# facebookresearch/CODD

Hardware: AMD Instinct MI355X
Metric: frames/sec full CODD forward @960x540 (whole job) (higher is better)
Workload: dtype f32 (split-bf16 MFMA operands, f32 accumulate; HITNet + context network + Fusion exact f32); 1 GPU; full CODD (HITNetMF + Motion/RAFT3D iters=16 + Fusion) 960x540 padded to 960x576, max_disp=320, one video per GPU, steady-state frames (idx>=1), synthetic stereo sequence, random-init weights; conv_precision=split, hip_graph=True, frames_per_gpu=311, prewarm_frames=150, side_streams=True, library=codd_amd/csrc/libcodd_hip.so, full=False

## Files before the change

### codd_amd/_abi.py

```python
import ctypes as C
import os

from . import build as _build

c_float_p = C.POINTER(C.c_float)


class View(C.Structure):
    _fields_ = [("ptr", C.c_void_p), ("ctot", C.c_int), ("coff", C.c_int)]


class XsView(C.Structure):
    _fields_ = [("ptr", C.c_void_p), ("c8", C.c_int), ("hp", C.c_int), ("wp", C.c_int), ("bt", C.c_int),
                ("bl", C.c_int), ("o8", C.c_int), ("terms", C.c_int)]


class ConvParams(C.Structure):
    _fields_ = [
        ("in0", View), ("in1", View), ("C0", C.c_int), ("C1", C.c_int),
        ("B", C.c_int), ("Hin", C.c_int), ("Win", C.c_int),
        ("wpacked", C.c_void_p), ("bias", C.c_void_p),
        ("res1", View), ("res2", View), ("post", View),
        ("out", C.c_void_p), ("out_ctot", C.c_int), ("out_coff", C.c_int),
        ("Cout", C.c_int), ("Hout", C.c_int), ("Wout", C.c_int),
        ("kh", C.c_int), ("kw", C.c_int), ("sy", C.c_int), ("sx", C.c_int),
        ("pad_t", C.c_int), ("pad_l", C.c_int), ("dil_y", C.c_int), ("dil_x", C.c_int),
        ("act", C.c_int), ("store_mode", C.c_int), ("mb", C.c_int), ("npb", C.c_int), ("nw", C.c_int), ("ck", C.c_int), ("layout", C.c_int),
        ("terms", C.c_int), ("pgw", C.c_int), ("cgw", C.c_int),
        ("xs", C.c_void_p), ("xs_c8", C.c_int), ("xs_hp", C.c_int), ("xs_wp", C.c_int),
        ("xs_bt", C.c_int), ("xs_bl", C.c_int), ("xs_o8", C.c_int),
        ("xso", C.c_void_p), ("xso_c8", C.c_int), ("xso_hp", C.c_int), ("xso_wp", C.c_int), ("xso_bt", C.c_int),
        ("xso_bl", C.c_int), ("xso_o8", C.c_int), ("xso_terms", C.c_int), ("ksplit", C.c_int), ("dil2", C.c_int), ("gate", C.c_int),
    ]


ACT = dict(none=0, lrelu=1, relu=2, sigmoid=3, tanh=4, mish=5, relu_ch0=6)




class RollParams(C.Structure):
    _fields_ = [("in0", View), ("in1", View), ("C0", C.c_int), ("C1", C.c_int),
                ("B", C.c_int), ("H", C.c_int), ("W", C.c_int), ("C", C.c_int), ("mode", C.c_int),
                ("wA", C.c_void_p), ("bA", C.c_void_p), ("wB", C.c_void_p), ("bB", C.c_void_p),
                ("actA", C.c_int), ("actB", C.c_int), ("residual", C.c_int),
                ("out", C.c_void_p), ("out_ctot", C.c_int), ("out_coff", C.c_int), ("cout_store", C.c_int),
                ("rh", C.c_int)]


_i, _f, _p, _ll = C.c_int, C.c_float, C.c_void_p, C.c_longlong

SIGNATURES = {
    "codd_abi_version": (_i, []),
    "codd_conv2d": (_i, [C.POINTER(ConvParams), _p]),
    "codd_conv2d_check": (_i, [C.POINTER(ConvParams)]),
    "codd_conv2d_multi": (_i, [C.POINTER(ConvParams), _i, _p]),
    "codd_roll_packed_size": (_ll, [_i, _i, _i]),
    "codd_roll_pack_weights": (_i, [_p, _p, _i, _i, _i, _i, _p]),
    "codd_conv_roll": (_i, [C.POINTER(RollParams), _p]),
    "codd_conv2d_packed_size": (_ll, [_i] * 6),
    "codd_conv2d_pack_weights": (_i, [_p, _p, _i, _i, _i, _i, _i, _i, _p]),
    "codd_tile_costvol_argmin": (_i, [_p, _p, _i, _i, _i, _i, _i, _i, _p, _i, _i, _p, _i, _i, _i, _p]),
    "codd_tile_warp_cost": (_i, [_p, _p, _i, _i, _i, _i, View, View, _i, _p, _p, _p]),
    "codd_hyp_upsample": (_i, [View, _i, _i, _i, _f, _p, _i, _i, _p]),
    "codd_hyp_select": (_i, [_p, View, View, _i, _i, _i, _p, _i, _i, _p]),
    "codd_instnorm": (_i, [_p, _i, _i, _i, _p, _p, _i, _p, _p]),
    "codd_instnorm_xs": (_i, [_p, _i, _i, _i, _i, _p, _p, _i, _i, _p, XsView, _p]),
    "codd_conv2d_pack_weights_ex": (_i, [_p, _p, _i, _i, _i, _i, _i, _i, _ll, _ll, _f, _p]),
    "codd_allpairs_corr": (_i, [_p, _p, _i, _i, _i, _i, _p, _p, _p, _p, _p, _p]),
    "codd_allpairs_corr_scratch": (_ll, [_i, _i, _i, _i]),
    "codd_avgpool2": (_i, [_p, _i, _i, _i, _p, _p]),
    "codd_induced_flow": (_i, [_p, _p, _i, _i, _i, _f, _f, _f, _f, _p, _p]),
    "codd_context_split": (_i, [_p, _i, _i, _p, _p, _p]),
    "codd_se3_identity": (_i, [_p, _ll, _p]),
    "codd_corr_lookup": (_i, [_p, _p, _p, _p, _p, _i, _i, _i, _i, _p, _p]),
    "codd_raft_geometry": (_i, [_p, _p, _p, _i, _i, _i, _f, _f, _f, _f, _p, _p, _p]),
    "codd_se3_gn_step": (_i, [_p, _p, _i, _p, _p, _p, _p, _i, _i, _i, _f, _f, _f, _f, _i, _f, _f, _p, _p]),
    "codd_se3_gn_scratch": (_ll, [_i, _i, _i, _i]),
    "codd_set_option": (_i, [_i, _i]),
    "codd_get_option": (_i, [_i]),
    "codd_se3_gn_step_heads": (_i, [_p, XsView, _p, _p, _p, _p, _i, _i, _i, _f, _f, _f, _f, _i, _f, _f, _p, _p, _p]),
    "codd_cvx_upsample": (_i, [_p, _p, _i, _i, _i, _i, _i, _p, _p]),
    "codd_cvx_upsample_se3_weight": (_i, [_p, _p, _p, _i, _i, _i, _p, _p, _p]),
    "codd_disp_to_depth": (_i, [_p, _ll, _f, _p, _p]),
    "codd_subsample": (_i, [_p, _i, _i, _i, _i, _i, _i, _p, _p]),
    "codd_splat": (_i, [_p, _p, _i, _i, _i, _i, _i, _p, _i, _p, _i, _i, _i, _i, _i, _f, _f, _f, _f, _f, _f,
                        _p, _p, _p, _p]),
    "codd_splat_scratch": (_ll, [_i, _i, _i, _f]),
    "codd_resize_bilinear": (_i, [_p, _i, _i, _i, _i, _i, _i, _i, _p, _i, _i, _i, _i, _p]),
    "codd_resize_bilinear_add": (_i, [_p, _i, _i, _i, _i, _i, _i, _i, _p, _i, _i, _i, _i, _p, _p]),
    "codd_add_relu": (_i, [_p, _p, _ll, _i, _p, _p]),
    "codd_copy_many": (_i, [_p, _p, _p, _i, _p]),
    "codd_timestamp": (_i, [_p, _p]),
    "codd_gru_gate_zr": (_i, [_p, _p, _p, _p, _p, _p, _i, _i, _p, _p, _p]),
    "codd_gru_gate_q": (_i, [_p, _p, _p, _p, _p, _p, _p, _i, _i, _p, _p]),
    "codd_gru_gate_zr_xs": (_i, [_p, _p, _p, _p, _p, _p, _i, _i, _i, _p, XsView, _p]),
    "codd_gru_gate_q_xs": (_i, [_p, _p, _p, _p, _p, _p, _p, _i, _i, _i, _p, XsView, _p]),
    "codd_fusion_cues_lr": (_i, [_p] * 6 + [_i] * 7 + [_p, _p, _i, _i, _p]),
    "codd_fusion_cues_fr": (_i, [_p, _p, _p, _p, _i, _i, _i, _i, _p, _p]),
    "codd_fusion_forget": (_i, [_p, _p, _p, _p, _i, _i, _i, _i, _p, _p, _p]),
    "codd_disp_metrics": (_i, [_p, _p, _i, _i, _i, _i, _i, _f, _f, _f, _p, _p, _p]),
    "codd_raft_geometry_lookup": (_i, [_p, _p, _p, _p, _p, _p, _p, _i, _i, _i, _f, _f, _f, _f, _p, _p, _p, _p]),
    "codd_raft_geometry_lookup_xs": (_i, [_p, _p, _p, _p, _p, _p, _p, _i, _i, _i, _f, _f, _f, _f, _p, XsView, XsView, _p]),
    "codd_conv2d_packed_size_quad": (C.c_longlong, [_i, _i, _i, _i, _i, _i]),
    "codd_conv2d_pack_weights_quad": (_i, [_p, _p, _i, _i, _i, _i, _i, _i, _p]),
    "codd_split_bf16_bytes": (_ll, [_i] * 5),
    "codd_split_bf16": (_i, [View, _i, View, _i, _i, _i, _i, _i, _i, _i, _i, _i, _i, _p, _p]),
    "codd_conv2d_packed_bytes_bf16": (_ll, [_i] * 7),
    "codd_conv2d_pack_weights_bf16": (_i, [_p, _p, _i, _i, _i, _i, _i, _i, _i, _ll, _ll, _f, _p]),
    "codd_fusion_select": (_i, [_i, _p, _p, _p, _i, _i, _i, _i, _i, _f, _p, _p]),
    "codd_gt_motion": (_i, [_p, _p, _p, _i, _p, _p, _p, _i, _i, _i, _i, _i, _p, _p, _p, _p, _p, _p]),
    "codd_tepe_metrics": (_i, [_p, _p, _p, _p, _p, _p, _p, _i, _i, _i, _i, _i, _f, _f, _f, _p, _p, _p]),
    "codd_sceneflow_metrics": (_i, [_p] * 6 + [_i] * 5 + [_f] * 7 + [_p, _p, _p]),
    "codd_preprocess": (_i, [_p, _i, _i, _i, C.POINTER(C.c_float), C.POINTER(C.c_float), _i, _i, _p, _p]),
    "codd_fusion_blend": (_i, [_p, _p, _p, _p, _i, _i, _i, _i, _p, _p, _p, _p]),
}

ABI_VERSION = 12
_lib = None
LOADED = None
MISSING = []


class CoddHipError(RuntimeError):
    pass


def lib_path():
    ab = os.environ.get("CODD_LIB_AB")
    if ab:
        import sys
        print(f"codd_amd: WARNING: CODD_LIB_AB is set -- loading the prebuilt {ab} instead of the in-tree library; it is NOT "
              f"checked against the sources of this tree", file=sys.stderr, flush=True)
        return ab
    return _build.LIB


def load():
    global _lib, LOADED
    if _lib is not None:
        return _lib
    path = lib_path()
    if path == _build.LIB and (not os.path.exists(path) or _build.needs_build()):
        import fcntl
        try:
            lock = open(os.path.join(os.path.dirname(path), ".build.lock"), "w")
        except OSError as e:
            raise CoddHipError(f"libcodd_hip.so is missing or older than its sources and {os.path.dirname(path)} is "
                               f"not writable: {e}") from e
        with lock:
            fcntl.flock(lock, fcntl.LOCK_EX)
            try:
                if not os.path.exists(path) or _build.needs_build():
                    try:
                        _build.build(verbose=False)
                    except Exception as e:
                        raise CoddHipError(f"libcodd_hip.so is missing or older than its sources and the rebuild "
                                           f"failed: {e}") from e
            finally:
                fcntl.flock(lock, fcntl.LOCK_UN)
    lib = C.CDLL(path)
    for name, (res, args) in SIGNATURES.items():
        try:
            fn = getattr(lib, name)
        except AttributeError:
            MISSING.append(name)
            continue
        fn.restype = res
        fn.argtypes = args
    if lib.codd_abi_version() != ABI_VERSION:
        raise CoddHipError("ABI version mismatch")
    _lib, LOADED = lib, path
    return lib


OPTIONS = dict(gn_q4=0, gn_builder=1)


def set_option(name, value):
    rc = load().codd_set_option(OPTIONS[name], int(value))
    if rc < 0:
        raise CoddHipError(f"codd_set_option({name}, {value}) rejected")
    return rc


def check(rc, what):
    if rc != 0:
        raise CoddHipError(f"{what} failed with code {rc}")
```

### codd_amd/csrc/conv.hip

```cpp
#include "conv_quad_kernel.h"
#include <stdio.h>
#include <stdlib.h>

CONV_ALL_GROUPS(CONV_DECLARE)
CONVQ_ALL(CONVQ_DECLARE)
CONVQ_MULTI(CONVQM_DECLARE)


__global__ void conv_pack_kernel(const float* __restrict__ w, float* __restrict__ wp, int Cout, int Cin, int ntaps,
                                 int mb, int ck, int wrow, int nchunks, long long total, long long co_stride,
                                 long long ci_stride, float scale) {
  long long e = (long long)blockIdx.x * blockDim.x + threadIdx.x;
  if (e >= total) return;
  int col = (int)(e % wrow);
  long long t = e / wrow;
  int c = (int)(t % ck); t /= ck;
  int tap = (int)(t % ntaps); t /= ntaps;
  int chunk = (int)(t % nchunks);
  int cog = (int)(t / nchunks);
  int co = cog * 16 * mb + col, ci = chunk * ck + c;
  float v = 0.f;
  if (col < 16 * mb && co < Cout && ci < Cin) v = w[(size_t)co * co_stride + (size_t)ci * ci_stride + tap] * scale;
  wp[e] = v;
}

__global__ void conv_pack_quad_kernel(const float* __restrict__ w, float* __restrict__ wp, int Cout, int Cin, int ntaps,
                                      int mb, int ck, int nchunks, long long total) {
  long long e = (long long)blockIdx.x * blockDim.x + threadIdx.x;
  if (e >= total) return;
  const int q = (int)(e & 3);
  long long t = e >> 2;
  const int col = (int)(t % (16 * mb)); t /= 16 * mb;
  const int cq = (int)(t % (ck >> 2)); t /= ck >> 2;
  const int tap = (int)(t % ntaps); t /= ntaps;
  const int chunk = (int)(t % nchunks);
  const int cog = (int)(t / nchunks);
  const int co = cog * 16 * mb + col, ci = chunk * ck + 4 * cq + q;
  wp[e] = (co < Cout && ci < Cin) ? w[((size_t)co * Cin + ci) * ntaps + tap] : 0.f;
}

extern "C" long long codd_conv2d_packed_size_quad(int Cout, int Cin, int kh, int kw, int mb, int ck) {
  if (mb < 1 || !(ck == 16 || ck == 32)) return -1;
  return (long long)cdiv(Cout, 16 * mb) * cdiv(Cin, ck) * (kh * kw) * ck * 16 * mb;
}

extern "C" int codd_conv2d_pack_weights_quad(const float* w, float* wpacked, int Cout, int Cin, int kh, int kw, int mb,
                                             int ck, void* stream) {
  const long long total = codd_conv2d_packed_size_quad(Cout, Cin, kh, kw, mb, ck);
  if (total <= 0 || !w || !wpacked) return CODD_EINVAL;
  conv_pack_quad_kernel<<<cdiv(total, 256), 256, 0, (hipStream_t)stream>>>(w, wpacked, Cout, Cin, kh * kw, mb, ck,
                                                                           cdiv(Cin, ck), total);
  CODD_LAUNCH_CHECK();
  return CODD_OK;
}

static inline int wrow_of(int mb) { return 16 * mb + ((mb & 1) ? 0 : 16); }

extern "C" long long codd_conv2d_packed_size(int Cout, int Cin, int kh, int kw, int mb, int ck) {
  if (mb < 1 || ck < 4 || (ck & 3)) return -1;
  long long ncog = cdiv(Cout, 16 * mb), nchunks = cdiv(Cin, ck);
  return ncog * nchunks * (long long)(kh * kw) * ck * wrow_of(mb);
}

extern "C" int codd_conv2d_pack_weights_ex(const float* w, float* wpacked, int Cout, int Cin, int kh, int kw, int mb,
                                           int ck, long long co_stride, long long ci_stride, float scale,
                                           void* stream) {
  long long total = codd_conv2d_packed_size(Cout, Cin, kh, kw, mb, ck);
  if (total <= 0 || !w || !wpacked) return CODD_EINVAL;
  int nchunks = cdiv(Cin, ck);
  conv_pack_kernel<<<cdiv(total, 256), 256, 0, (hipStream_t)stream>>>(w, wpacked, Cout, Cin, kh * kw, mb, ck,
                                                                      wrow_of(mb), nchunks, total, co_stride,
                                                                      ci_stride, scale);
  CODD_LAUNCH_CHECK();
  return CODD_OK;
}

extern "C" int codd_conv2d_pack_weights(const float* w, float* wpacked, int Cout, int Cin, int kh, int kw, int mb,
                                        int ck, void* stream) {
  return codd_conv2d_pack_weights_ex(w, wpacked, Cout, Cin, kh, kw, mb, ck, (long long)Cin * kh * kw,
                                     (long long)kh * kw, 1.f, stream);
}

template <int NW, int NPB, int MB, int WREG, int IREG>
static int launch_conv(const ConvK& k, size_t lds, int grid, hipStream_t s) {
  if (lds > 64 * 1024) {
    hipError_t e = hipFuncSetAttribute((const void*)conv_mfma_kernel<NW, NPB, MB, WREG, IREG>,
                                       hipFuncAttributeMaxDynamicSharedMemorySize, (int)lds);
    if (e != hipSuccess) return (int)e;
  }
  conv_mfma_kernel<NW, NPB, MB, WREG, IREG><<<grid, NW * 64, lds, s>>>(k);
  CODD_LAUNCH_CHECK();
  return CODD_OK;
}

template <int NPB, int MB>
static int launch_conv_regs(const ConvK& k, size_t lds, int grid, hipStream_t s) {
  const int wr = cdiv(k.wchunk >> 2, 256), ir = cdiv(k.nunits, 256);
  if (wr <= 4 && ir <= 4) return launch_conv<4, NPB, MB, 4, 4>(k, lds, grid, s);
  if (wr <= 4 && ir <= 8) return launch_conv<4, NPB, MB, 4, 8>(k, lds, grid, s);
  if (wr <= 12 && ir <= 4) return launch_conv<4, NPB, MB, 12, 4>(k, lds, grid, s);
  if (wr <= 12 && ir <= 8) return launch_conv<4, NPB, MB, 12, 8>(k, lds, grid, s);
  if (wr <= 16 && ir <= 8) return launch_conv<4, NPB, MB, 16, 8>(k, lds, grid, s);
  return CODD_EUNSUPPORTED;
}

template <int NW, int MB>
static int launch_conv_nwx(const ConvK& k, size_t lds, int grid, hipStream_t s) {
  const int wr = cdiv(k.wchunk >> 2, NW * 64), ir = cdiv(k.nunits, NW * 64);
  if (wr <= 8 && ir <= 4) return launch_conv<NW, 1, MB, 8, 4>(k, lds, grid, s);
  if (wr <= 16 && ir <= 4) return launch_conv<NW, 1, MB, 16, 4>(k, lds, grid, s);
  return CODD_EUNSUPPORTED;
}

template <int NW, int NPB, int MB, int WREG, int QREG>
static int launch_quad(const ConvK& k, size_t lds, int grid, hipStream_t s) {
  if (lds > 64 * 1024) {
    hipError_t e = hipFuncSetAttribute((const void*)conv_quad_kernel<NW, NPB, MB, WREG, QREG>,
                                       hipFuncAttributeMaxDynamicSharedMemorySize, (int)lds);
    if (e != hipSuccess) return (int)e;
  }
  conv_quad_kernel<NW, NPB, MB, WREG, QREG><<<grid, NW * 64, lds, s>>>(k);
  CODD_LAUNCH_CHECK();
  return CODD_OK;
}

static int launch_quad_any(const ConvK& k, int nw, size_t lds, int grid, hipStream_t s) {
  const codd_conv_params& p = k.p;
  const int nt = nw * 64, wr = cdiv(k.wchunk >> 2, nt), qr = cdiv((p.ck >> 2) * k.upc, nt);
#define Q(W, N, M, R, QQ) if (nw == W && p.npb == N && p.mb == M && wr <= R && qr <= QQ) return launch_quad<W, N, M, R, QQ>(k, lds, grid, s);
  Q(4, 1, 1, 8, 2) Q(4, 1, 2, 8, 1) Q(4, 1, 2, 16, 2) Q(4, 1, 4, 12, 1) Q(4, 1, 4, 16, 2)
  Q(4, 2, 1, 8, 2) Q(4, 2, 2, 8, 2) Q(4, 2, 2, 16, 2) Q(4, 2, 4, 12, 2) Q(4, 2, 4, 16, 2)
  Q(4, 4, 1, 8, 4) Q(4, 4, 2, 8, 4)
  Q(9, 1, 1, 8, 1) Q(9, 1, 2, 8, 1) Q(9, 1, 4, 8, 1) Q(9, 1, 4, 16, 1)
#undef Q
  return CODD_EUNSUPPORTED;
}

int codd_conv2d_bf16(const codd_conv_params* pp, void* stream, int dry_run);

extern "C" int codd_conv2d_check(const codd_conv_params* pp) {
  if (!pp || pp->layout != 2) return CODD_EINVAL;
  return codd_conv2d_bf16(pp, nullptr, 1);
}

static int conv_fill(const codd_conv_params* pp, ConvK& k, size_t& lds, long long& grid, int& nw) {
  k.p = *pp;
  const codd_conv_params& p = k.p;
  if (!p.in0.ptr || !p.out || !p.wpacked || p.C0 <= 0 || p.C1 < 0 || (p.C1 > 0 && !p.in1.ptr)) return CODD_EINVAL;
  if (p.ck < 4 || (p.ck & 3) || p.B < 1 || p.Cout < 1 || p.kh < 1 || p.kw < 1 || p.pad_l < 0 || p.pad_t < 0)
    return CODD_EINVAL;
  if (!(p.mb == 1 || p.mb == 2 || p.mb == 4) || !(p.npb == 1 || p.npb == 2 || p.npb == 4)) return CODD_EINVAL;
  if (p.store_mode && (p.kh != 1 || p.kw != 1 || p.res1.ptr || p.res2.ptr || p.post.ptr)) return CODD_EUNSUPPORTED;
  k.cin = p.C0 + p.C1;
  k.nchunks = cdiv(k.cin, p.ck);
  k.ntaps = p.kh * p.kw;
  const int xb = p.npb >= 2 ? 2 : 1, rpw = p.npb / xb;
  nw = p.nw ? p.nw : 4;
  if (nw != 4 && (!(nw == 9 || nw == 2 || nw == 8) || p.npb != 1)) return CODD_EUNSUPPORTED;
  k.th = nw * rpw;
  k.tw = 16 * xb;
  k.thi = (k.th - 1) * p.sy + (p.kh - 1) * p.dil_y + 1;
  k.twi = (k.tw - 1) * p.sx + (p.kw - 1) * p.dil_x + 1;
  k.xoff = (4 - (p.pad_l % 4)) % 4;
  k.twp = ((k.xoff + k.twi + 3) / 4) * 4;
  k.twp4 = k.twp / 4;
  k.upc = k.thi * k.twp4;
  k.nunits = p.ck * k.upc;
  const int per = k.thi * k.twp;
  if (p.sx == 1) k.chs = ((per + 15) / 32) * 32 + 16;
  else k.chs = per + 4;
  k.wrow = wrow_of(p.mb);
  k.wchunk = k.ntaps * p.ck * k.wrow;
  k.tiles_x = cdiv(p.Wout, k.tw);
  k.tiles_y = cdiv(p.Hout, k.th);
  k.cout_eff = p.store_mode ? 4 * p.Cout : p.Cout;
  k.ncog = cdiv(k.cout_eff, 16 * p.mb);
  const size_t hwb = (size_t)p.Hin * p.Win * sizeof(float);
  k.vec_ok = (p.Win % 4 == 0) && ((uintptr_t)p.in0.ptr % 16 == 0) && (hwb % 16 == 0) &&
             (p.C1 == 0 || (uintptr_t)p.in1.ptr % 16 == 0);
  lds = ((size_t)k.wchunk + (size_t)p.ck * k.chs) * sizeof(float);
  if (p.layout == 1) {
    if (!(p.ck == 16 || p.ck == 32) || p.sx > 2 || !k.vec_ok) return CODD_EUNSUPPORTED;
    k.wchunk = k.ntaps * p.ck * 16 * p.mb;
    lds = ((size_t)k.wchunk + (size_t)p.ck * k.thi * k.twp) * sizeof(float);
  } else if (p.layout != 0) {
    return CODD_EINVAL;
  }
  if (lds > 160 * 1024) return CODD_EUNSUPPORTED;
  grid = (long long)k.tiles_x * k.tiles_y * k.ncog * p.B;
  if (grid <= 0 || grid > 0x7fffffffLL) return CODD_EINVAL;
  k.xcd = 1;
  return CODD_OK;
}

extern "C" int codd_conv2d(const codd_conv_params* pp, void* stream) {
  if (!pp) return CODD_EINVAL;
  if (pp->layout != 2 && (pp->dil2 || pp->gate)) return CODD_EUNSUPPORTED;
  if (pp->layout == 2) {
    const codd_conv_params& q = *pp;
    if (!q.xs || (!q.out && !q.xso) || !q.wpacked || q.C0 <= 0 || q.C1 < 0 || q.B < 1 || q.Cout < 1 || q.kh < 1 || q.kw < 1 ||
        q.pad_l < 0 || q.pad_t < 0)
      return CODD_EINVAL;
    if (q.store_mode && (q.kh != 1 || q.kw != 1 || q.res1.ptr || q.res2.ptr || q.post.ptr)) return CODD_EUNSUPPORTED;
    return codd_conv2d_bf16(pp, stream, 0);
  }
  ConvK k;
  size_t lds;
  long long grid;
  int nw;
  const int rc = conv_fill(pp, k, lds, grid, nw);
  if (rc != CODD_OK) return rc;
  const codd_conv_params& p = k.p;
  hipStream_t s = (hipStream_t)stream;
  if (p.layout == 1) return launch_quad_any(k, nw, lds, (int)grid, s);
#define CASEW(W, M) if (nw == W && p.mb == M) return launch_conv_nwx<W, M>(k, lds, (int)grid, s)
  CASEW(9, 1); CASEW(9, 2); CASEW(9, 4); CASEW(2, 1); CASEW(2, 2); CASEW(2, 4); CASEW(8, 1); CASEW(8, 2); CASEW(8, 4);
#undef CASEW
#define CASE(N, M) if (p.npb == N && p.mb == M) return launch_conv_regs<N, M>(k, lds, (int)grid, s)
  CASE(1, 1); CASE(1, 2); CASE(1, 4);
  CASE(2, 1); CASE(2, 2); CASE(2, 4);
  CASE(4, 1); CASE(4, 2); CASE(4, 4);
#undef CASE
  return CODD_EUNSUPPORTED;
}

template <int NW, int NPB, int MB, int WREG, int QREG>
static int launch_quad_multi(const ConvKN& kn, size_t lds, int grid, hipStream_t s) {
  if (lds > 64 * 1024) {
    hipError_t e = hipFuncSetAttribute((const void*)conv_quad_multi_kernel<NW, NPB, MB, WREG, QREG>,
                                       hipFuncAttributeMaxDynamicSharedMemorySize, (int)lds);
    if (e != hipSuccess) return (int)e;
  }
  conv_quad_multi_kernel<NW, NPB, MB, WREG, QREG><<<grid, NW * 64, lds, s>>>(kn);
  CODD_LAUNCH_CHECK();
  return CODD_OK;
}

extern "C" int codd_conv2d_multi(const codd_conv_params* ps, int n, void* stream) {
  if (!ps || n < 1 || n > CONVQ_MULTI_MAX) return CODD_EINVAL;
  if (n == 1) return codd_conv2d(ps, stream);
  ConvKN kn;
  memset(&kn, 0, sizeof(kn));
  size_t lds = 0;
  long long total = 0;
  int wr = 0, qr = 0;
  for (int i = 0; i < n; ++i) {
    size_t l;
    long long g;
    int nw;
    if (ps[i].layout != 1) return CODD_EUNSUPPORTED;
    const int rc = conv_fill(&ps[i], kn.k[i], l, g, nw);
    if (rc != CODD_OK) return rc;
    const codd_conv_params& p = kn.k[i].p;
    if (nw != 4 || p.npb != 1 || p.mb != ps[0].mb || !(p.mb == 1 || p.mb == 2)) return CODD_EUNSUPPORTED;
    const int w_ = cdiv(kn.k[i].wchunk >> 2, 256), q_ = cdiv((p.ck >> 2) * kn.k[i].upc, 256);
    wr = w_ > wr ? w_ : wr;
    qr = q_ > qr ? q_ : qr;
    lds = l > lds ? l : lds;
    kn.start[i] = (int)total;
    total += g;
  }
  for (int i = n; i <= CONVQ_MULTI_MAX; ++i) kn.start[i] = (int)total;
  if (total > 0x7fffffffLL) return CODD_EINVAL;
  hipStream_t s = (hipStream_t)stream;
  if (ps[0].mb == 1 && wr <= 8 && qr <= 2) return launch_quad_multi<4, 1, 1, 8, 2>(kn, lds, (int)total, s);
  if (ps[0].mb == 2 && wr <= 16 && qr <= 2) return launch_quad_multi<4, 1, 2, 16, 2>(kn, lds, (int)total, s);
  return CODD_EUNSUPPORTED;
}

extern "C" int codd_avgpool2(const float* in, int BC, int h, int w, float* out, void* stream);

#define CORR_MB 4
#define CORR_CK 32
extern "C" long long codd_allpairs_corr_scratch(int B, int D, int h, int w) {
  long long packed = codd_conv2d_packed_size(h * w, D, 1, 1, CORR_MB, CORR_CK);
  long long pooled = 0;
  int hh = h, ww = w;
  for (int i = 1; i < 4; ++i) { hh >>= 1; ww >>= 1; pooled += (long long)D * hh * ww; }
  return (long long)B * (packed + pooled);
}

extern "C" int codd_allpairs_corr(const float* f1, const float* f2, int B, int D, int h, int w, float* lvl0,
                                  float* lvl1, float* lvl2, float* lvl3, float* scratch, void* stream) {
  if (!f1 || !f2 || !lvl0 || !lvl1 || !lvl2 || !lvl3 || !scratch || (h >> 3) < 1 || (w >> 3) < 1) return CODD_EINVAL;
  const int N = h * w;
  const long long packed = codd_conv2d_packed_size(N, D, 1, 1, CORR_MB, CORR_CK);
  float* lv[4] = {lvl0, lvl1, lvl2, lvl3};
  for (int b = 0; b < B; ++b) {
    float* wp = scratch + (size_t)b * packed;
    int rc = codd_conv2d_pack_weights_ex(f1 + (size_t)b * D * N, wp, N, D, 1, 1, CORR_MB, CORR_CK, 1, N, 1.f / 16.f,
                                         stream);
    if (rc) return rc;
  }
  float* pool = scratch + (size_t)B * packed;
  const float* src = f2;
  int hh = h, ww = w;
  for (int i = 0; i < 4; ++i) {
    if (i > 0) {
      int rc = codd_avgpool2(src, B * D, hh, ww, pool, stream);
      if (rc) return rc;
      src = pool;
      hh >>= 1; ww >>= 1;
      pool += (size_t)B * D * hh * ww;
    }
    for (int b = 0; b < B; ++b) {
      codd_conv_params p;
      memset(&p, 0, sizeof(p));
      p.in0.ptr = src + (size_t)b * D * hh * ww; p.in0.ctot = D; p.in0.coff = 0;
      p.C0 = D; p.C1 = 0; p.B = 1; p.Hin = hh; p.Win = ww;
      p.wpacked = scratch + (size_t)b * packed;
      p.out = lv[i] + (size_t)b * N * hh * ww; p.out_ctot = N; p.out_coff = 0;
      p.Cout = N; p.Hout = hh; p.Wout = ww;
      p.kh = p.kw = 1; p.sy = p.sx = 1; p.dil_y = p.dil_x = 1;
      p.act = CODD_ACT_NONE; p.mb = CORR_MB; p.ck = CORR_CK;
      p.npb = 1;
      int rc = codd_conv2d(&p, stream);
      if (rc) return rc;
    }
  }
  return CODD_OK;
}
```

### codd_amd/csrc/conv_bf16_kernel.h

```cpp
#pragma once
#include <stdlib.h>
#include "conv_kernel.h"

typedef __bf16 bf16x8 __attribute__((ext_vector_type(8)));
typedef _Float16 f16x8 __attribute__((ext_vector_type(8)));

struct ConvB {
  codd_conv_params p;
  int cin, nchunks, ntaps, noct;
  int nk;
  int th, tw, thi, twi;
  int pu, xb;
  int npix;
  int xplane;
  int nring;
  int os16;
  int iplane16;
  int ibuf16;
  int wplane16;
  int nco;
  int wslots;
  int tiles_x, tiles_y, ncog, cout_eff;
  int khe;
  unsigned m_iplane16, m_os16, m_twi, m_noct, m_kw;
};
static inline unsigned convb_magic(int d) { return d <= 1 ? 0u : (unsigned)((0x100000000ULL + (unsigned)d - 1) / (unsigned)d); }
__device__ __forceinline__ int convb_div(int n, unsigned M, int d) { return d == 1 ? n : (int)__umulhi((unsigned)n, M); }

constexpr int CONVB_NWP = 4;
constexpr int CONVB_MAXP = 6;
#ifdef CONVB_NO_DMA
#define CONVB_DMA_N(n) 0
#else
#define CONVB_DMA_N(n) (n)
#endif
#ifdef CONVB_NO_INPUT
#define CONVB_IN_N(n) 0
#else
#define CONVB_IN_N(n) (n)
#endif

static inline int convb_geometry(const codd_conv_params* pp, ConvB& k, size_t& lds, long long& grid, bool need_xs) {
  k.p = *pp;
  const codd_conv_params& p = k.p;
  if (p.ck < 8 || (p.ck & 7) || !CODD_TERMS_OK(p.terms) || p.nw < 1 || p.npb < 1 || p.npb > 2 ||
      p.pgw < 1 || p.cgw < 1 || p.mb < 1 || p.mb % p.cgw)
    return CODD_EINVAL;
  const int planes = CODD_TERMS_PLANES(p.terms);
  k.cin = p.C0 + p.C1;
  k.ntaps = p.kh * p.kw;
  k.noct = p.ck >> 3;
  k.nchunks = cdiv(k.cin, p.ck);
  k.nk = cdiv((long long)k.ntaps * k.noct, 4);
  k.th = p.nw; k.xb = p.npb; k.pu = k.th * k.xb; k.tw = 16 * k.xb;
  if (p.dil2 < 0 || (p.dil2 > 0 && ((p.kh & 1) || !(p.kh / 2 & 1) || !(p.kw & 1) || p.dil2 > p.dil_y || p.dil2 > p.dil_x)))
    return CODD_EINVAL;
  k.khe = p.dil2 > 0 ? p.kh / 2 : p.kh;
  k.thi = (k.th - 1) * p.sy + (k.khe - 1) * p.dil_y + 1;
  k.twi = (k.tw - 1) * p.sx + (p.kw - 1) * p.dil_x + 1;
  k.npix = k.thi * k.twi;
  k.os16 = ((k.npix + 15) / 16) * 16;
  while ((planes * k.noct * k.os16) & 63) k.os16 += 16;
  k.iplane16 = k.noct * k.os16;
  k.ibuf16 = planes * k.iplane16;
  k.nco = 16 * p.mb;
  k.wplane16 = k.nk * 4 * k.nco;
  k.wslots = planes * k.wplane16;
  k.tiles_x = cdiv(p.Wout, k.tw);
  k.tiles_y = cdiv(p.Hout, k.th);
  k.cout_eff = p.store_mode ? 4 * p.Cout : p.Cout;
  k.ncog = cdiv(k.cout_eff, k.nco);
  const size_t per = ((size_t)k.wslots + (size_t)k.ibuf16) * 16, tab = ((size_t)k.nk + 2) * 16;
  k.nring = (k.nchunks >= 3 && 3 * per + tab <= 160 * 1024) ? 3 : 2;
  lds = k.nring * per + tab;
  if (lds > 160 * 1024) return CODD_EUNSUPPORTED;
  if (p.ksplit < 0 || p.ksplit > 2) return CODD_EINVAL;
  if (p.ksplit == 2 && (size_t)cdiv(k.pu, p.pgw) * p.mb * p.pgw * 1024 > k.nring * per) return CODD_EUNSUPPORTED;
  if ((k.nring - 1) * (cdiv(k.wslots >> 6, CONVB_NWP) + cdiv(k.ibuf16 >> 6, CONVB_NWP)) > 56) return CODD_EUNSUPPORTED;
  k.xplane = p.xs_c8 * p.xs_hp * p.xs_wp;
  if (k.nring * (k.wslots + k.ibuf16) + 64 >= 65536 || (k.nk + 2) * 4 >= 65536) return CODD_EUNSUPPORTED;
  k.m_iplane16 = convb_magic(k.iplane16); k.m_os16 = convb_magic(k.os16); k.m_twi = convb_magic(k.twi);
  k.m_noct = convb_magic(k.noct); k.m_kw = convb_magic(p.kw);
  if (need_xs && (!p.xs || p.xs_o8 < 0 || p.xs_c8 < p.xs_o8 + k.nchunks * k.noct || p.xs_bt < p.pad_t ||
                  p.xs_bl < p.pad_l || p.xs_hp < p.xs_bt + p.Hin || p.xs_wp < p.xs_bl + p.Win ||
                  p.xs_hp < p.xs_bt - p.pad_t + (k.tiles_y * k.th - 1) * p.sy + (k.khe - 1) * p.dil_y + 1 ||
                  p.xs_wp < p.xs_bl - p.pad_l + (k.tiles_x * k.tw - 1) * p.sx + (p.kw - 1) * p.dil_x + 1))
    return CODD_EINVAL;
  if (p.gate < 0 || p.gate > 3) return CODD_EINVAL;
  if (need_xs && p.gate) {
    const int G = p.gate == 2 ? k.cout_eff / 3 : k.cout_eff;
    auto c4ok = [](const codd_view& v, int need) {
      return v.ptr && !((uintptr_t)v.ptr & 15) && !(v.ctot & 3) && !(v.coff & 3) && v.coff >= 0 && v.coff + need <= v.ctot;
    };
    if (p.store_mode || (G & 15) || (p.gate == 2 && 3 * G != k.cout_eff)) return CODD_EUNSUPPORTED;
    if (!p.out || ((uintptr_t)p.out & 15) || (p.out_ctot & 3) || (p.out_coff & 3) ||
        p.out_coff + (p.gate == 2 ? 2 * G : G) > p.out_ctot || (p.bias && ((uintptr_t)p.bias & 15)))
      return CODD_EINVAL;
    if (p.gate == 1 && (p.xso || p.res1.ptr || p.res2.ptr || p.post.ptr)) return CODD_EUNSUPPORTED;
    if (p.gate == 2 && (!p.xso || !c4ok(p.res1, 3 * G) || !c4ok(p.res2, 2 * G) || !c4ok(p.post, G))) return CODD_EINVAL;
    if (p.gate == 3 && (!p.xso || !c4ok(p.res1, 2 * G) || !c4ok(p.post, G) || p.res2.ptr)) return CODD_EINVAL;
    if (p.xso && (p.xso_terms != p.terms || p.xso_o8 < 0 || p.xso_bt < 0 || p.xso_bl < 0 ||
                  p.xso_c8 < p.xso_o8 + cdiv(G, 8) || p.xso_hp < p.xso_bt + p.Hout || p.xso_wp < p.xso_bl + p.Wout))
      return CODD_EINVAL;
  } else if (need_xs && p.xso) {
    if (p.store_mode || p.res1.ptr || p.res2.ptr || p.post.ptr || p.act == CODD_ACT_RELU_CH0) return CODD_EUNSUPPORTED;
    if (p.bias && ((uintptr_t)p.bias & 15)) return CODD_EINVAL;
    if (p.xso_terms != p.terms || p.xso_o8 < 0 || p.xso_bt < 0 || p.xso_bl < 0 ||
        p.xso_c8 < p.xso_o8 + cdiv(k.cout_eff, 8) || p.xso_hp < p.xso_bt + p.Hout || p.xso_wp < p.xso_bl + p.Wout)
      return CODD_EINVAL;
  }
  grid = (long long)k.tiles_x * k.tiles_y * k.ncog * p.B;
  if (grid <= 0 || grid > 0x7fffffffLL) return CODD_EINVAL;
  return CODD_OK;
}

__device__ __attribute__((noinline)) f32x4 convb_act_slow(f32x4 v, int act) {
#pragma unroll
  for (int r = 0; r < 4; ++r) v[r] = act_apply(v[r], act, 1);
  return v;
}
__device__ __forceinline__ f32x4 convb_act(f32x4 v, int act, int co) {
  if (act == CODD_ACT_NONE) return v;
  if (act == CODD_ACT_RELU || (act == CODD_ACT_RELU_CH0 && co == 0)) {
#pragma unroll
    for (int r = 0; r < 4; ++r) v[r] = fmaxf(v[r], 0.f);
    return v;
  }
  if (act == CODD_ACT_RELU_CH0) return v;
  if (act == CODD_ACT_LRELU02) {
#pragma unroll
    for (int r = 0; r < 4; ++r) v[r] = v[r] > 0.f ? v[r] : 0.2f * v[r];
    return v;
  }
  return convb_act_slow(v, act);
}

__device__ __forceinline__ void convb_wait_vmcnt(int n) {
#define CONVB_W1(N) case N: asm volatile("s_waitcnt vmcnt(" #N ")" ::: "memory"); break;
#define CONVB_W8(N) CONVB_W1(N) CONVB_W1(N + 1) CONVB_W1(N + 2) CONVB_W1(N + 3) CONVB_W1(N + 4) CONVB_W1(N + 5) CONVB_W1(N + 6) CONVB_W1(N + 7)
  switch (n) {
    CONVB_W8(0) CONVB_W8(8) CONVB_W8(16) CONVB_W8(24) CONVB_W8(32) CONVB_W8(40) CONVB_W8(48)
    default: break;
  }
#undef CONVB_W8
#undef CONVB_W1
}

__device__ __forceinline__ void convb_dma16(const uint4* gsrc, unsigned lds_dst) {
  unsigned keep;
  asm volatile("s_mov_b32 %0, m0\n\ts_mov_b32 m0, %2\n\ts_nop 0\n\tglobal_load_lds_dwordx4 %1, off\n\ts_mov_b32 m0, %0"
               : "=&s"(keep) : "v"(gsrc), "s"(lds_dst) : "memory");
}

template <int I, int NR, int NM>
struct ConvbSched {
  static __device__ __forceinline__ void run() {
    constexpr int q = ((I + 1) * NM) / NR - (I * NM) / NR;
    if constexpr (q > 0) __builtin_amdgcn_sched_group_barrier(0x008, q, 0);
    __builtin_amdgcn_sched_group_barrier(0x100, 1, 0);
    if constexpr (I + 1 < NR) ConvbSched<I + 1, NR, NM>::run();
  }
};

template <int PGW, int CGW, int A, int B, int TERMS, int OUTF, int KS>
__global__ __launch_bounds__((PGW * CGW * KS + CONVB_NWP) * 64) void conv_bf16_kernel(const ConvB k) {
  constexpr int NWT = PGW * CGW;
  constexpr int NWC = NWT * KS;
  constexpr int NTP = CONVB_NWP * 64;
  constexpr int NPL = CODD_TERMS_PLANES(TERMS);
  constexpr bool F16 = CODD_TERMS_IS_F16(TERMS);
  extern __shared__ __attribute__((aligned(16))) uint4 smem4[];
  uint4* wl = smem4;
  uint4* il = smem4 + k.nring * k.wslots;
  int* etab = (int*)(il + k.nring * k.ibuf16);
  const codd_conv_params& p = k.p;
  const int tid = threadIdx.x, lane = tid & 63;
  const int wave = __builtin_amdgcn_readfirstlane(tid >> 6);

  int bid = blockIdx.x;
  const int tx = bid % k.tiles_x; bid /= k.tiles_x;
  const int ty = bid % k.tiles_y; bid /= k.tiles_y;
  const int cog = bid % k.ncog;
  const int b = bid / k.ncog;

  if (wave >= NWC) {
    const int pt = tid - NWC * 64;
    const int pw = wave - NWC;
    const int nwv = k.wslots >> 6, niv = k.ibuf16 >> 6;
    const int nd = (nwv - pw + CONVB_NWP - 1) / CONVB_NWP + (niv - pw + CONVB_NWP - 1) / CONVB_NWP;
    const unsigned wl_lds = (unsigned)(uintptr_t)(__attribute__((address_space(3))) uint4*)wl;
    const unsigned il_lds = (unsigned)(uintptr_t)(__attribute__((address_space(3))) uint4*)il;
#define BF_DMA_W(CH, BUF)                                                                                 \
  {                                                                                                       \
    const uint4* wsrc_ = (const uint4*)p.wpacked + ((size_t)(cog * k.nchunks + (CH))) * k.wslots + lane;  \
    const unsigned wdst_ = wl_lds + (unsigned)(BUF) * (unsigned)k.wslots * 16u;                           \
    for (int i_ = pw; i_ < nwv; i_ += CONVB_NWP)                                                          \
      convb_dma16(wsrc_ + i_ * 64, __builtin_amdgcn_readfirstlane(wdst_ + (unsigned)i_ * 1024u));         \
  }
#ifndef CONVB_NO_PRODUCER
    BF_DMA_W(0, 0);
#endif
    const int oct_rec = p.xs_hp * p.xs_wp;
    const uint4* xs0 = (const uint4*)p.xs + (size_t)b * NPL * k.xplane + (size_t)p.xs_o8 * oct_rec +
                       (size_t)(ty * k.th * p.sy + p.xs_bt - p.pad_t) * p.xs_wp + tx * k.tw * p.sx + p.xs_bl - p.pad_l;
    auto piece_off = [&](int i_) -> int {
      const int s_ = i_ * 64 + lane;
      const int pl_ = convb_div(s_, k.m_iplane16, k.iplane16), r_ = s_ - pl_ * k.iplane16;
      const int oc_ = convb_div(r_, k.m_os16, k.os16);
      int px_ = r_ - oc_ * k.os16;
      px_ = px_ < k.npix ? px_ : 0;
      const int y_ = convb_div(px_, k.m_twi, k.twi), x_ = px_ - y_ * k.twi;
      return pl_ * k.xplane + oc_ * oct_rec + y_ * p.xs_wp + x_;
    };
    int ioff[CONVB_MAXP];
#pragma unroll
    for (int q_ = 0; q_ < CONVB_MAXP; ++q_) ioff[q_] = piece_off(pw + q_ * CONVB_NWP);
#define BF_DMA_I(CH, BUF)                                                                                 \
  {                                                                                                       \
    const uint4* xsrc_ = xs0 + (size_t)(CH) * k.noct * oct_rec;                                           \
    const unsigned idst_ = il_lds + (unsigned)(BUF) * (unsigned)k.ibuf16 * 16u;                           \
    _Pragma("unroll") for (int q_ = 0; q_ < CONVB_MAXP; ++q_) {                                           \
      const int i_ = pw + q_ * CONVB_NWP;                                                                 \
      if (i_ < niv) convb_dma16(xsrc_ + ioff[q_], __builtin_amdgcn_readfirstlane(idst_ + (unsigned)i_ * 1024u)); \
    }                                                                                                     \
    for (int i_ = pw + CONVB_MAXP * CONVB_NWP; i_ < niv; i_ += CONVB_NWP)                                 \
      convb_dma16(xsrc_ + piece_off(i_), __builtin_amdgcn_readfirstlane(idst_ + (unsigned)i_ * 1024u));   \
  }
#define BF_DMA(CH, BUF) { BF_DMA_W(CH, BUF) BF_DMA_I(CH, BUF) }
#ifndef CONVB_NO_PRODUCER
    const int ahead = k.nring - 1;
    BF_DMA_I(0, 0);
    if (ahead > 1 && k.nchunks > 1) BF_DMA(1, 1);
#endif
    for (int e = pt; e < (k.nk + 2) * 4; e += NTP) {
      const int tap = convb_div(e, k.m_noct, k.noct), oct = e - tap * k.noct;
      int off = 0;
      if (e < k.nk * 4 && tap < k.ntaps) {
        const int ky = convb_div(tap, k.m_kw, p.kw), kx = tap - ky * p.kw;
        if (p.dil2 > 0 && ky < k.khe)
          off = oct * k.os16 + ((k.khe >> 1) * (p.dil_y - p.dil2) + ky * p.dil2) * k.twi +
                (p.kw >> 1) * (p.dil_x - p.dil2) + kx * p.dil2;
        else
          off = oct * k.os16 + (ky - (p.dil2 > 0 ? k.khe : 0)) * p.dil_y * k.twi + kx * p.dil_x;
      }
      etab[e] = off;
    }
#ifndef CONVB_NO_PRODUCER
    convb_wait_vmcnt(ahead > 1 && k.nchunks > 1 ? nd : 0);
    asm volatile("s_waitcnt lgkmcnt(0)" ::: "memory");
    __builtin_amdgcn_s_barrier();
    int slot = ahead == k.nring ? 0 : ahead;
    for (int c = 0; c < k.nchunks; ++c) {
      if (c + ahead < k.nchunks) BF_DMA(c + ahead, slot);
      slot = slot + 1 == k.nring ? 0 : slot + 1;
      int fly_ = k.nchunks - (c + 2);
      fly_ = fly_ < 0 ? 0 : (fly_ > ahead - 1 ? ahead - 1 : fly_);
      convb_wait_vmcnt(fly_ * nd);
      __builtin_amdgcn_s_barrier();
    }
#endif
#undef BF_DMA
#undef BF_DMA_W
#undef BF_DMA_I
    return;
  }

  const int g = lane >> 4, j = lane & 15;
  const int kpart = KS == 1 ? 0 : wave / NWT, wset = KS == 1 ? wave : wave - kpart * NWT;
  const int cgi = wset % CGW, pgi = wset / CGW;
  f32x4 acc[A][B];
#pragma unroll
  for (int a = 0; a < A; ++a)
#pragma unroll
    for (int m = 0; m < B; ++m) acc[a][m] = (f32x4){0.f, 0.f, 0.f, 0.f};

  int pbase[A];
#pragma unroll
  for (int a = 0; a < A; ++a) {
    int u = pgi * A + a;
    if (u >= k.pu) u = k.pu - 1;
    const int prow = u / k.xb, pcol = (u - prow * k.xb) * 16 + j;
    pbase[a] = prow * p.sy * k.twi + pcol * p.sx;
  }
  const int woff = g * k.nco + cgi * B * 16 + j;
  const int wstep = 4 * k.nco;

  struct Frag { bf16x8 ah[B], al[B], bh[A], bl[A]; };
#define BF_LOAD(F, KSTP)                                                                                   \
  {                                                                                                       \
    const int eo_ = eo;                                                                                   \
    eo = etab[((KSTP) + KS) * 4 + g];                                                                   \
    const uint4* wp_ = wb + woff + (KSTP) * wstep;                                                          \
    _Pragma("unroll") for (int m_ = 0; m_ < B; ++m_) {                                                    \
      F.ah[m_] = __builtin_bit_cast(bf16x8, wp_[m_ * 16]);                                                \
      if (NPL == 2) F.al[m_] = __builtin_bit_cast(bf16x8, wp_[k.wplane16 + m_ * 16]);                   \
    }                                                                                                     \
    _Pragma("unroll") for (int a_ = 0; a_ < A; ++a_) {                                                    \
      F.bh[a_] = __builtin_bit_cast(bf16x8, ib[eo_ + pbase[a_]]);                                         \
      if (NPL == 2) F.bl[a_] = __builtin_bit_cast(bf16x8, ib[k.iplane16 + eo_ + pbase[a_]]);            \
    }                                                                                                     \
  }
  auto mma = [](bf16x8 x, bf16x8 y, f32x4 c) -> f32x4 {
    if constexpr (F16)
      return __builtin_amdgcn_mfma_f32_16x16x32_f16(__builtin_bit_cast(f16x8, x), __builtin_bit_cast(f16x8, y), c, 0, 0, 0);
    else
      return __builtin_amdgcn_mfma_f32_16x16x32_bf16(x, y, c, 0, 0, 0);
  };
#define BF_MFMA(F)                                                                                        \
  {                                                                                                       \
    if (NPL == 2) {                                                                                       \
      _Pragma("unroll") for (int a = 0; a < A; ++a) _Pragma("unroll") for (int m = 0; m < B; ++m)         \
        acc[a][m] = OUTF ? mma(F.al[m], F.bh[a], acc[a][m]) : mma(F.bh[a], F.al[m], acc[a][m]);           \
      _Pragma("unroll") for (int a = 0; a < A; ++a) _Pragma("unroll") for (int m = 0; m < B; ++m)         \
        acc[a][m] = OUTF ? mma(F.ah[m], F.bl[a], acc[a][m]) : mma(F.bl[a], F.ah[m], acc[a][m]);           \
    }                                                                                                     \
    _Pragma("unroll") for (int a = 0; a < A; ++a) _Pragma("unroll") for (int m = 0; m < B; ++m)           \
      acc[a][m] = OUTF ? mma(F.ah[m], F.bh[a], acc[a][m]) : mma(F.bh[a], F.ah[m], acc[a][m]);             \
  }

  __syncthreads();
#ifndef CONVB_NO_CONSUMER
  const int klast = k.nk - 1;
  constexpr int NRD = 1 + NPL * (A + B), NMF = (NPL == 2 ? 3 : 1) * A * B;
  int wsel = 0;
  for (int ch = 0; ch < k.nchunks; ++ch) {
    const uint4* wb = wl + wsel * k.wslots;
    const uint4* ib = il + wsel * k.ibuf16;
    wsel = wsel + 1 == k.nring ? 0 : wsel + 1;
    const int kfirst = KS == 1 ? 0 : ((kpart + ch) & 1);
    if (KS == 1 || kfirst < k.nk) {
      const int mylast = KS == 1 ? klast : kfirst + ((klast - kfirst) / KS) * KS;
      Frag f0, f1;
      int eo = etab[kfirst * 4 + g];
      BF_LOAD(f0, kfirst);
      int ks = kfirst;
      for (; ks + KS < k.nk; ks += 2 * KS) {
#ifdef CONVB_NO_LDSREAD
        if (ch == 0 && ks == kfirst)
#endif
        BF_LOAD(f1, ks + KS);
        BF_MFMA(f0);
#ifndef CONVB_NO_SCHED
        ConvbSched<0, NRD, NMF>::run();
#endif
#ifdef CONVB_NO_LDSREAD
        if (ch == 0 && ks == kfirst)
#endif
        BF_LOAD(f0, ks + 2 * KS < mylast ? ks + 2 * KS : mylast);
        BF_MFMA(f1);
#ifndef CONVB_NO_SCHED
        ConvbSched<0, NRD, NMF>::run();
#endif
      }
      if (ks < k.nk) BF_MFMA(f0);
    }
#ifndef CONVB_NO_BARRIER
    __syncthreads();
#endif
  }
#endif
#undef BF_LOAD
#undef BF_MFMA
  if constexpr (KS == 2) {
    f32x4* red = (f32x4*)smem4 + (size_t)wset * (A * B) * 64 + lane;
#pragma unroll
    for (int a = 0; a < A; ++a)
#pragma unroll
      for (int m = 0; m < B; ++m)
        if (((a * B + m) & 1) != kpart) red[(a * B + m) * 64] = acc[a][m];
    __syncthreads();
#pragma unroll
    for (int a = 0; a < A; ++a)
#pragma unroll
      for (int m = 0; m < B; ++m)
        if (((a * B + m) & 1) == kpart) acc[a][m] += red[(a * B + m) * 64];
  }

#ifdef CONVB_NO_EPILOGUE
  {
    float s_ = 0.f;
#pragma unroll
    for (int a = 0; a < A; ++a)
#pragma unroll
      for (int m = 0; m < B; ++m) s_ += acc[a][m][0] + acc[a][m][1] + acc[a][m][2] + acc[a][m][3];
    p.out[(size_t)blockIdx.x * 256 + tid] = s_;
    return;
  }
#endif
  if constexpr (OUTF == 1) {
    const int orec = p.xso_hp * p.xso_wp;
    uint4* xo = (uint4*)p.xso + (size_t)b * NPL * p.xso_c8 * orec;
    const bool odd = g & 1;
#pragma unroll
    for (int a = 0; a < A; ++a) {
      const int u = pgi * A + a;
      const int prow = u / k.xb;
      const int oy = ty * k.th + prow;
      const int ox = tx * k.tw + (u - prow * k.xb) * 16 + j;
      const bool inb = u < k.pu && oy < p.Hout && ox < p.Wout;
#pragma unroll
      for (int m = 0; m < B; ++m) {
        if (KS == 2 && ((a * B + m) & 1) != kpart) continue;
        const int co0 = (cog * CGW * B + cgi * B + m) * 16 + 4 * g;
        f32x4 v = acc[a][m];
        if (p.bias) {
          if (co0 + 3 < k.cout_eff) v += *(const f32x4*)(p.bias + co0);
          else
#pragma unroll
            for (int r = 0; r < 4; ++r) v[r] += co0 + r < k.cout_eff ? p.bias[co0 + r] : 0.f;
        }
        int rco = co0;
        if (p.gate) {
          const int hw_ = p.Hout * p.Wout, pix_ = oy * p.Wout + ox;
          auto c4 = [&](const float* base, int ctot, int c) {
            return (f32x4*)(base + (((size_t)b * (ctot >> 2) + (c >> 2)) * hw_ + pix_) * 4);
          };
          const bool live = inb && co0 < k.cout_eff;
          const int ctile = co0 & ~15;
          if (p.gate == 1) {
            if (live) *c4(p.out, p.out_ctot, p.out_coff + co0) = v;
            continue;
          }
          const int G = p.gate == 2 ? k.cout_eff / 3 : k.cout_eff;
          if (p.gate == 2) {
            if (live) v += *c4(p.res1.ptr, p.res1.ctot, p.res1.coff + co0);
            if (ctile >= 2 * G) {
              if (live) *c4(p.out, p.out_ctot, p.out_coff + co0 - G) = v;
              continue;
            }
            if (live) v += *c4(p.res2.ptr, p.res2.ctot, p.res2.coff + co0);
            v = convb_act_slow(v, CODD_ACT_SIGMOID);
            if (ctile < G) {
              if (live) *c4(p.out, p.out_ctot, p.out_coff + co0) = v;
              continue;
            }
            rco = co0 - G;
            if (live) v *= *c4(p.post.ptr, p.post.ctot, p.post.coff + rco);
          } else {
            f32x4 z = f32x4{0.f, 0.f, 0.f, 0.f}, h = z;
            if (live) {
              v += *c4(p.res1.ptr, p.res1.ctot, p.res1.coff + G + co0);
              z = *c4(p.res1.ptr, p.res1.ctot, p.res1.coff + co0);
              h = *c4(p.post.ptr, p.post.ctot, p.post.coff + co0);
            }
            v = convb_act_slow(v, CODD_ACT_TANH);
#pragma unroll
            for (int r = 0; r < 4; ++r) v[r] = (1.f - z[r]) * h[r] + z[r] * v[r];
            if (live) *c4(p.out, p.out_ctot, p.out_coff + co0) = v;
          }
        } else {
          v = convb_act(v, p.act, 1);
        }
#pragma unroll
        for (int r = 0; r < 4; ++r) v[r] = co0 + r < k.cout_eff ? v[r] : 0.f;
        unsigned hi2[2], lo2[2];
#pragma unroll
        for (int q = 0; q < 2; ++q) {
          if constexpr (F16) {
            const _Float16 h0 = (_Float16)v[2 * q], h1 = (_Float16)v[2 * q + 1];
            const _Float16 l0 = (_Float16)(v[2 * q] - (float)h0), l1 = (_Float16)(v[2 * q + 1] - (float)h1);
            hi2[q] = (unsigned)__builtin_bit_cast(unsigned short, h0) | ((unsigned)__builtin_bit_cast(unsigned short, h1) << 16);
            lo2[q] = (unsigned)__builtin_bit_cast(unsigned short, l0) | ((unsigned)__builtin_bit_cast(unsigned short, l1) << 16);
          } else {
            const __bf16 h0 = (__bf16)v[2 * q], h1 = (__bf16)v[2 * q + 1];
            const __bf16 l0 = (__bf16)(v[2 * q] - (float)h0), l1 = (__bf16)(v[2 * q + 1] - (float)h1);
            hi2[q] = (unsigned)__builtin_bit_cast(unsigned short, h0) | ((unsigned)__builtin_bit_cast(unsigned short, h1) << 16);
            lo2[q] = (unsigned)__builtin_bit_cast(unsigned short, l0) | ((unsigned)__builtin_bit_cast(unsigned short, l1) << 16);
          }
        }
        const unsigned s0 = odd ? hi2[0] : lo2[0], s1 = odd ? hi2[1] : lo2[1];
        const unsigned r0 = __shfl_xor(s0, 16, 64), r1 = __shfl_xor(s1, 16, 64);
        const uint4 rec = odd ? make_uint4(r0, r1, lo2[0], lo2[1]) : make_uint4(hi2[0], hi2[1], r0, r1);
        const int oct = (rco >> 3) + p.xso_o8;
        if (inb && (co0 & ~7) < k.cout_eff && (!odd || NPL == 2))
          xo[(size_t)(odd ? p.xso_c8 * orec : 0) + ((size_t)oct * p.xso_hp + oy + p.xso_bt) * p.xso_wp + ox + p.xso_bl] = rec;
      }
    }
    return;
  }
  const int hwout = p.Hout * p.Wout;
  const bool vec = (p.Wout & 3) == 0 && p.store_mode == 0;
#pragma unroll
  for (int a = 0; a < A; ++a) {
    const int u = pgi * A + a;
    if (u >= k.pu) continue;
    const int prow = u / k.xb;
    const int oy = ty * k.th + prow;
    const int ox = tx * k.tw + (u - prow * k.xb) * 16 + 4 * g;
    if (oy >= p.Hout || ox >= p.Wout) continue;
    const int pix = oy * p.Wout + ox;
#pragma unroll
    for (int m = 0; m < B; ++m) {
      if (KS == 2 && ((a * B + m) & 1) != kpart) continue;
      const int co = (cog * CGW * B + cgi * B + m) * 16 + j;
      if (co >= k.cout_eff) continue;
      f32x4 v = acc[a][m];
      if (p.store_mode == 0) {
        if (p.bias) v += p.bias[co];
        float* op = p.out + ((size_t)b * p.out_ctot + p.out_coff + co) * (size_t)hwout + pix;
        if (vec) {
          if (p.res1.ptr) v += *(const f32x4*)(view_ptr(p.res1, b, co, hwout) + pix);
          if (p.res2.ptr) v += *(const f32x4*)(view_ptr(p.res2, b, co, hwout) + pix);
          v = convb_act(v, p.act, co);
          if (p.post.ptr) v += *(const f32x4*)(view_ptr(p.post, b, co, hwout) + pix);
#if defined(CONVB_NT_STORE)
          __builtin_nontemporal_store(v, (f32x4*)op);
#elif defined(CONVB_SC1_STORE)
          asm volatile("global_store_dwordx4 %0, %1, off sc1" ::"v"(op), "v"(v) : "memory");
#else
          *(f32x4*)op = v;
#endif
        } else {
#pragma unroll
          for (int r = 0; r < 4; ++r)
            if (ox + r < p.Wout) {
              if (p.res1.ptr) v[r] += view_ptr(p.res1, b, co, hwout)[pix + r];
              if (p.res2.ptr) v[r] += view_ptr(p.res2, b, co, hwout)[pix + r];
            }
          v = convb_act(v, p.act, co);
#pragma unroll
          for (int r = 0; r < 4; ++r)
            if (ox + r < p.Wout) op[r] = v[r] + (p.post.ptr ? view_ptr(p.post, b, co, hwout)[pix + r] : 0.f);
        }
      } else {
        const int q = co / p.Cout, c = co - q * p.Cout;
        if (p.bias) v += p.bias[c];
        v = convb_act(v, p.act, c);
        const int W2 = 2 * p.Wout;
        float* op = p.out + ((size_t)b * p.out_ctot + p.out_coff + c) * (size_t)(4 * hwout) +
                    (size_t)(2 * oy + (q >> 1)) * W2 + (q & 1);
#pragma unroll
        for (int r = 0; r < 4; ++r)
          if (ox + r < p.Wout) op[2 * (ox + r)] = v[r];
      }
    }
  }
}

#define CONVB_GROUP_A(X) X(2, 2, 5, 2, 1)
#define CONVB_GROUP_B(X) X(4, 1, 4, 4, 1)
#define CONVB_GROUP_C(X) X(4, 1, 4, 2, 1)
#define CONVB_GROUP_D(X) X(4, 1, 4, 1, 1) X(4, 1, 8, 1, 1)
#define CONVB_GROUP_E(X) X(4, 1, 2, 2, 1) X(4, 1, 2, 1, 1)
#define CONVB_GROUP_F(X) X(4, 1, 3, 4, 1) X(4, 1, 3, 2, 1)
#define CONVB_GROUP_G(X) X(2, 2, 5, 2, 2)
#define CONVB_GROUP_H(X) X(4, 1, 4, 2, 2)
#define CONVB_GROUP_I(X) X(4, 1, 3, 2, 2) X(4, 1, 3, 4, 2)
#define CONVB_GROUP_J(X) X(4, 2, 4, 2, 1)
#define CONVB_GROUP_K(X) X(4, 2, 3, 2, 1)
#define CONVB_GROUP_L(X) X(8, 1, 4, 4, 1)
#define CONVB_ALL(X)                                                                                   \
  CONVB_GROUP_A(X) CONVB_GROUP_B(X) CONVB_GROUP_C(X) CONVB_GROUP_D(X) CONVB_GROUP_E(X) CONVB_GROUP_F(X) \
  CONVB_GROUP_G(X) CONVB_GROUP_H(X) CONVB_GROUP_I(X) CONVB_GROUP_J(X) CONVB_GROUP_K(X) CONVB_GROUP_L(X)
#define CONVB_DECLARE(PGW, CGW, A, B, KS)                                                        \
  extern template __global__ void conv_bf16_kernel<PGW, CGW, A, B, 1, 0, KS>(const ConvB);      \
  extern template __global__ void conv_bf16_kernel<PGW, CGW, A, B, 3, 0, KS>(const ConvB);      \
  extern template __global__ void conv_bf16_kernel<PGW, CGW, A, B, 1, 1, KS>(const ConvB);      \
  extern template __global__ void conv_bf16_kernel<PGW, CGW, A, B, 3, 1, KS>(const ConvB);      \
  extern template __global__ void conv_bf16_kernel<PGW, CGW, A, B, 16, 0, KS>(const ConvB);     \
  extern template __global__ void conv_bf16_kernel<PGW, CGW, A, B, 16, 1, KS>(const ConvB);     \
  extern template __global__ void conv_bf16_kernel<PGW, CGW, A, B, 48, 0, KS>(const ConvB);     \
  extern template __global__ void conv_bf16_kernel<PGW, CGW, A, B, 48, 1, KS>(const ConvB);
#define CONVB_DEFINE(PGW, CGW, A, B, KS)                                                         \
  template __global__ void conv_bf16_kernel<PGW, CGW, A, B, 1, 0, KS>(const ConvB);             \
  template __global__ void conv_bf16_kernel<PGW, CGW, A, B, 3, 0, KS>(const ConvB);             \
  template __global__ void conv_bf16_kernel<PGW, CGW, A, B, 1, 1, KS>(const ConvB);             \
  template __global__ void conv_bf16_kernel<PGW, CGW, A, B, 3, 1, KS>(const ConvB);             \
  template __global__ void conv_bf16_kernel<PGW, CGW, A, B, 16, 0, KS>(const ConvB);            \
  template __global__ void conv_bf16_kernel<PGW, CGW, A, B, 16, 1, KS>(const ConvB);            \
  template __global__ void conv_bf16_kernel<PGW, CGW, A, B, 48, 0, KS>(const ConvB);            \
  template __global__ void conv_bf16_kernel<PGW, CGW, A, B, 48, 1, KS>(const ConvB);
```

### codd_amd/csrc/conv_kernel.h

```cpp
#pragma once
#include "common.h"
#include <stdint.h>
#include <string.h>


struct ConvK {
  codd_conv_params p;
  int cin, nchunks, ntaps;
  int th, tw, thi, twi, chs;
  int wrow, wchunk;
  int tiles_x, tiles_y, ncog;
  int cout_eff;
  int twp;
  int xoff;
  int twp4;
  int upc;
  int nunits;
  int vec_ok;
  int xcd;
};

__device__ __forceinline__ int conv_xcd_item(int bid, int nwg) {
  const int q = nwg >> 3, r = nwg & 7, x = bid & 7, idx = bid >> 3;
  return (x < r ? x * (q + 1) : r * (q + 1) + (x - r) * q) + idx;
}

__device__ __forceinline__ const float* view_ptr(const codd_view& v, int b, int c, int hw) {
  return v.ptr + ((size_t)b * v.ctot + v.coff + c) * (size_t)hw;
}

template <int NW, int NPB, int MB, int WREG, int IREG>
__global__ __launch_bounds__(NW * 64) void conv_mfma_kernel(const ConvK k) {
  constexpr int NT = NW * 64;
  extern __shared__ __attribute__((aligned(16))) float smem[];
  float* wl = smem;
  float* il = smem + k.wchunk;
  const codd_conv_params& p = k.p;
  const int tid = threadIdx.x, lane = tid & 63, wave = tid >> 6;
  const int g = lane >> 4, j = lane & 15;
  constexpr int XB = NPB >= 2 ? 2 : 1;
  constexpr int RPW = NPB / XB;

  int bid = k.xcd ? conv_xcd_item(blockIdx.x, gridDim.x) : blockIdx.x;
  const int tx = bid % k.tiles_x; bid /= k.tiles_x;
  const int ty = bid % k.tiles_y; bid /= k.tiles_y;
  const int cog = bid % k.ncog;
  const int b = bid / k.ncog;

  const int hwin = p.Hin * p.Win;
  const int gy0 = ty * k.th * p.sy - p.pad_t;
  const int gxs = tx * k.tw * p.sx - p.pad_l - k.xoff;

  int u_lds[IREG], u_g[IREG], u_c[IREG];
  unsigned u_m[IREG];
#pragma unroll
  for (int r = 0; r < IREG; ++r) {
    const int u = tid + r * NT;
    u_c[r] = -1; u_m[r] = 0; u_lds[r] = 0; u_g[r] = 0;
    if (u < k.nunits) {
      const int c = u / k.upc, rem = u - c * k.upc;
      const int y = rem / k.twp4, x4 = rem - y * k.twp4;
      const int gy = gy0 + y, gx = gxs + 4 * x4;
      unsigned m = 0;
      if ((unsigned)gy < (unsigned)p.Hin) {
#pragma unroll
        for (int q = 0; q < 4; ++q) m |= ((unsigned)(gx + q) < (unsigned)p.Win) ? (1u << q) : 0u;
      }
      u_c[r] = c; u_m[r] = m;
      u_lds[r] = c * k.chs + y * k.twp + 4 * x4;
      u_g[r] = gy * p.Win + gx;
    }
  }
  const int wchunk4 = k.wchunk >> 2;
  float4 wreg[WREG], ireg[IREG];

#define CONV_ISSUE(CH)                                                                                    \
  {                                                                                                       \
    const float4* src_ = (const float4*)(p.wpacked + ((size_t)(cog * k.nchunks + (CH))) * k.wchunk);      \
    _Pragma("unroll") for (int r = 0; r < WREG; ++r) {                                                    \
      const int e = tid + r * NT;                                                                         \
      wreg[r] = e < wchunk4 ? src_[e] : make_float4(0.f, 0.f, 0.f, 0.f);                                  \
    }                                                                                                     \
    const int c0_ = (CH) * p.ck;                                                                          \
    _Pragma("unroll") for (int r = 0; r < IREG; ++r) {                                                    \
      float4 v = make_float4(0.f, 0.f, 0.f, 0.f);                                                         \
      const int cg = c0_ + u_c[r];                                                                        \
      if (u_c[r] >= 0 && cg < k.cin && u_m[r]) {                                                          \
        const float* s_ =                                                                                 \
            (cg < p.C0 ? view_ptr(p.in0, b, cg, hwin) : view_ptr(p.in1, b, cg - p.C0, hwin)) + u_g[r];    \
        if (u_m[r] == 0xFu && k.vec_ok) {                                                                 \
          v = *(const float4*)s_;                                                                         \
        } else {                                                                                          \
          if (u_m[r] & 1u) v.x = s_[0];                                                                   \
          if (u_m[r] & 2u) v.y = s_[1];                                                                   \
          if (u_m[r] & 4u) v.z = s_[2];                                                                   \
          if (u_m[r] & 8u) v.w = s_[3];                                                                   \
        }                                                                                                 \
      }                                                                                                   \
      ireg[r] = v;                                                                                        \
    }                                                                                                     \
  }
#define CONV_COMMIT()                                                                                     \
  {                                                                                                       \
    float4* dst_ = (float4*)wl;                                                                           \
    _Pragma("unroll") for (int r = 0; r < WREG; ++r) {                                                    \
      const int e = tid + r * NT;                                                                         \
      if (e < wchunk4) dst_[e] = wreg[r];                                                                 \
    }                                                                                                     \
    _Pragma("unroll") for (int r = 0; r < IREG; ++r) if (u_c[r] >= 0) *(float4*)(il + u_lds[r]) = ireg[r]; \
  }

  f32x4 acc[NPB][MB];
#pragma unroll
  for (int a = 0; a < NPB; ++a)
#pragma unroll
    for (int m = 0; m < MB; ++m) acc[a][m] = (f32x4){0.f, 0.f, 0.f, 0.f};

  int pbase[NPB];
#pragma unroll
  for (int a = 0; a < NPB; ++a) {
    const int prow = wave * RPW + a / XB, pcol = (a % XB) * 16 + j;
    pbase[a] = prow * p.sy * k.twp + pcol * p.sx + k.xoff;
  }

  CONV_ISSUE(0);
  for (int ch = 0; ch < k.nchunks; ++ch) {
    __syncthreads();
    CONV_COMMIT();
    __syncthreads();
    if (ch + 1 < k.nchunks) CONV_ISSUE(ch + 1);
    for (int ky = 0; ky < p.kh; ++ky) {
      for (int kx = 0; kx < p.kw; ++kx) {
        const float* wp = wl + (ky * p.kw + kx) * p.ck * k.wrow + j + g * k.wrow;
        const float* ip = il + ky * p.dil_y * k.twp + kx * p.dil_x + g * k.chs;
        const int wstep = 4 * k.wrow, istep = 4 * k.chs;
#pragma unroll 4
        for (int c4 = 0; c4 < p.ck; c4 += 4) {
          float av[MB], bv[NPB];
#pragma unroll
          for (int m = 0; m < MB; ++m) av[m] = wp[m * 16];
#pragma unroll
          for (int a = 0; a < NPB; ++a) bv[a] = ip[pbase[a]];
          wp += wstep;
          ip += istep;
#pragma unroll
          for (int a = 0; a < NPB; ++a)
#pragma unroll
            for (int m = 0; m < MB; ++m)
              acc[a][m] = __builtin_amdgcn_mfma_f32_16x16x4f32(av[m], bv[a], acc[a][m], 0, 0, 0);
        }
      }
    }
  }

  const int hwout = p.Hout * p.Wout;
#pragma unroll
  for (int a = 0; a < NPB; ++a) {
    const int oy = ty * k.th + wave * RPW + a / XB;
    const int ox = tx * k.tw + (a % XB) * 16 + j;
    if (oy >= p.Hout || ox >= p.Wout) continue;
    const int pix = oy * p.Wout + ox;
#pragma unroll
    for (int m = 0; m < MB; ++m) {
#pragma unroll
      for (int r = 0; r < 4; ++r) {
        const int co = (cog * MB + m) * 16 + 4 * g + r;
        if (co >= k.cout_eff) continue;
        float v = acc[a][m][r];
        if (p.store_mode == 0) {
          if (p.bias) v += p.bias[co];
          if (p.res1.ptr) v += view_ptr(p.res1, b, co, hwout)[pix];
          if (p.res2.ptr) v += view_ptr(p.res2, b, co, hwout)[pix];
          v = act_apply(v, p.act, co);
          if (p.post.ptr) v += view_ptr(p.post, b, co, hwout)[pix];
          p.out[((size_t)b * p.out_ctot + p.out_coff + co) * (size_t)hwout + pix] = v;
        } else {
          const int q = co / p.Cout, c = co - q * p.Cout;
          if (p.bias) v += p.bias[c];
          v = act_apply(v, p.act, c);
          const int W2 = 2 * p.Wout;
          p.out[((size_t)b * p.out_ctot + p.out_coff + c) * (size_t)(4 * hwout) +
                (size_t)(2 * oy + (q >> 1)) * W2 + 2 * ox + (q & 1)] = v;
        }
      }
    }
  }
}

#define CONV_REGS_NW4(X, NPB, MB) X(4, NPB, MB, 4, 4) X(4, NPB, MB, 4, 8) X(4, NPB, MB, 12, 4) X(4, NPB, MB, 12, 8) X(4, NPB, MB, 16, 8)
#define CONV_REGS_NWX(X, NW, MB) X(NW, 1, MB, 8, 4) X(NW, 1, MB, 16, 4)
#define CONV_GROUP_0(X) CONV_REGS_NW4(X, 1, 1)
#define CONV_GROUP_1(X) CONV_REGS_NW4(X, 1, 2)
#define CONV_GROUP_2(X) CONV_REGS_NW4(X, 1, 4)
#define CONV_GROUP_3(X) CONV_REGS_NW4(X, 2, 1) CONV_REGS_NW4(X, 2, 2)
#define CONV_GROUP_4(X) CONV_REGS_NW4(X, 2, 4) CONV_REGS_NW4(X, 4, 1)
#define CONV_GROUP_5(X) CONV_REGS_NW4(X, 4, 2)
#define CONV_GROUP_6(X) CONV_REGS_NW4(X, 4, 4)
#define CONV_GROUP_7(X) CONV_REGS_NWX(X, 9, 1) CONV_REGS_NWX(X, 9, 2) CONV_REGS_NWX(X, 9, 4)
#define CONV_GROUP_8(X) CONV_REGS_NWX(X, 2, 1) CONV_REGS_NWX(X, 2, 2) CONV_REGS_NWX(X, 2, 4)
#define CONV_GROUP_9(X) CONV_REGS_NWX(X, 8, 1) CONV_REGS_NWX(X, 8, 2) CONV_REGS_NWX(X, 8, 4)
#define CONV_ALL_GROUPS(X) CONV_GROUP_0(X) CONV_GROUP_1(X) CONV_GROUP_2(X) CONV_GROUP_3(X) CONV_GROUP_4(X) CONV_GROUP_5(X) CONV_GROUP_6(X) CONV_GROUP_7(X) CONV_GROUP_8(X) CONV_GROUP_9(X)
#define CONV_DECLARE(NW, NPB, MB, WREG, IREG) extern template __global__ void conv_mfma_kernel<NW, NPB, MB, WREG, IREG>(const ConvK);
#define CONV_DEFINE(NW, NPB, MB, WREG, IREG) template __global__ void conv_mfma_kernel<NW, NPB, MB, WREG, IREG>(const ConvK);
```

### codd_amd/csrc/conv_quad_kernel.h

```cpp
#pragma once
#include "conv_kernel.h"

template <int NW, int NPB, int MB, int WREG, int QREG>
__device__ __forceinline__ void conv_quad_body(const ConvK& k, int bid, float* smem) {
  constexpr int NT = NW * 64;
  float* wl = smem;
  float* il = smem + k.wchunk;
  const codd_conv_params& p = k.p;
  const int tid = threadIdx.x, lane = tid & 63, wave = tid >> 6;
  const int g = lane >> 4, j = lane & 15;
  constexpr int XB = NPB >= 2 ? 2 : 1;
  constexpr int RPW = NPB / XB;

  const int tx = bid % k.tiles_x; bid /= k.tiles_x;
  const int ty = bid % k.tiles_y; bid /= k.tiles_y;
  const int cog = bid % k.ncog;
  const int b = bid / k.ncog;

  const int hwin = p.Hin * p.Win;
  const int gy0 = ty * k.th * p.sy - p.pad_t;
  const int gxs = tx * k.tw * p.sx - p.pad_l - k.xoff;

  const int ncq = p.ck >> 2;
  const int nq = ncq * k.upc;
  int q_lds[QREG], q_g[QREG], q_c[QREG];
  bool q_in[QREG];
#pragma unroll
  for (int r = 0; r < QREG; ++r) {
    const int u = tid + r * NT;
    q_c[r] = -1; q_in[r] = false; q_lds[r] = 0; q_g[r] = 0;
    if (u < nq) {
      const int cq = u / k.upc, rem = u - cq * k.upc;
      const int y = rem / k.twp4, x4 = rem - y * k.twp4;
      const int gy = gy0 + y, gx = gxs + 4 * x4;
      q_c[r] = 4 * cq;
      q_in[r] = (unsigned)gy < (unsigned)p.Hin && gx >= 0 && gx + 3 < p.Win;
      q_lds[r] = ((cq * k.thi + y) * k.twp + 4 * x4) * 4;
      q_g[r] = gy * p.Win + gx;
    }
  }
  const int wchunk4 = k.wchunk >> 2;
  float4 wreg[WREG], ireg[QREG][4];

#define QUAD_ISSUE(CH)                                                                                    \
  {                                                                                                       \
    const float4* src_ = (const float4*)(p.wpacked + ((size_t)(cog * k.nchunks + (CH))) * k.wchunk);      \
    _Pragma("unroll") for (int r = 0; r < WREG; ++r) {                                                    \
      const int e = tid + r * NT;                                                                         \
      wreg[r] = e < wchunk4 ? src_[e] : make_float4(0.f, 0.f, 0.f, 0.f);                                  \
    }                                                                                                     \
    _Pragma("unroll") for (int r = 0; r < QREG; ++r) {                                                    \
      _Pragma("unroll") for (int c = 0; c < 4; ++c) {                                                     \
        float4 v = make_float4(0.f, 0.f, 0.f, 0.f);                                                       \
        const int cg = (CH) * p.ck + q_c[r] + c;                                                          \
        if (q_c[r] >= 0 && q_in[r] && cg < k.cin) {                                                       \
          const float* s_ =                                                                               \
              (cg < p.C0 ? view_ptr(p.in0, b, cg, hwin) : view_ptr(p.in1, b, cg - p.C0, hwin)) + q_g[r];  \
          v = *(const float4*)s_;                                                                         \
        }                                                                                                 \
        ireg[r][c] = v;                                                                                   \
      }                                                                                                   \
    }                                                                                                     \
  }
#define QUAD_COMMIT()                                                                                     \
  {                                                                                                       \
    float4* dst_ = (float4*)wl;                                                                           \
    _Pragma("unroll") for (int r = 0; r < WREG; ++r) {                                                    \
      const int e = tid + r * NT;                                                                         \
      if (e < wchunk4) dst_[e] = wreg[r];                                                                 \
    }                                                                                                     \
    _Pragma("unroll") for (int r = 0; r < QREG; ++r) if (q_c[r] >= 0) {                                   \
      float4* d_ = (float4*)(il + q_lds[r]);   \
      d_[0] = make_float4(ireg[r][0].x, ireg[r][1].x, ireg[r][2].x, ireg[r][3].x);                        \
      d_[1] = make_float4(ireg[r][0].y, ireg[r][1].y, ireg[r][2].y, ireg[r][3].y);                        \
      d_[2] = make_float4(ireg[r][0].z, ireg[r][1].z, ireg[r][2].z, ireg[r][3].z);                        \
      d_[3] = make_float4(ireg[r][0].w, ireg[r][1].w, ireg[r][2].w, ireg[r][3].w);                        \
    }                                                                                                     \
  }

  f32x4 acc[NPB][MB];
#pragma unroll
  for (int a = 0; a < NPB; ++a)
#pragma unroll
    for (int m = 0; m < MB; ++m) acc[a][m] = (f32x4){0.f, 0.f, 0.f, 0.f};

  int pbase[NPB];
#pragma unroll
  for (int a = 0; a < NPB; ++a) {
    const int prow = wave * RPW + a / XB, pcol = (a % XB) * 16 + j;
    pbase[a] = prow * p.sy * k.twp + pcol * p.sx + k.xoff;
  }
  const int wq = 16 * MB;
  const int iq = k.thi * k.twp;
  const int ngr = p.ck >> 4;

  QUAD_ISSUE(0);
  for (int ch = 0; ch < k.nchunks; ++ch) {
    __syncthreads();
    QUAD_COMMIT();
    __syncthreads();
    if (ch + 1 < k.nchunks) QUAD_ISSUE(ch + 1);
    const float4* w4 = (const float4*)wl;
    const float4* i4 = (const float4*)il;
    for (int ky = 0; ky < p.kh; ++ky) {
      for (int kx = 0; kx < p.kw; ++kx) {
        const float4* wp = w4 + ((size_t)(ky * p.kw + kx) * (p.ck >> 2) + g) * wq + j;
        const float4* ip = i4 + (size_t)g * iq + ky * p.dil_y * k.twp + kx * p.dil_x;
        for (int gr = 0; gr < ngr; ++gr) {
          float4 av[MB], bv[NPB];
#pragma unroll
          for (int m = 0; m < MB; ++m) av[m] = wp[m * 16];
#pragma unroll
          for (int a = 0; a < NPB; ++a) bv[a] = ip[pbase[a]];
          wp += 4 * wq;
          ip += 4 * iq;
#pragma unroll
          for (int a = 0; a < NPB; ++a)
#pragma unroll
            for (int m = 0; m < MB; ++m) {
              acc[a][m] = __builtin_amdgcn_mfma_f32_16x16x4f32(av[m].x, bv[a].x, acc[a][m], 0, 0, 0);
              acc[a][m] = __builtin_amdgcn_mfma_f32_16x16x4f32(av[m].y, bv[a].y, acc[a][m], 0, 0, 0);
              acc[a][m] = __builtin_amdgcn_mfma_f32_16x16x4f32(av[m].z, bv[a].z, acc[a][m], 0, 0, 0);
              acc[a][m] = __builtin_amdgcn_mfma_f32_16x16x4f32(av[m].w, bv[a].w, acc[a][m], 0, 0, 0);
            }
        }
      }
    }
  }
#undef QUAD_ISSUE
#undef QUAD_COMMIT

  const int hwout = p.Hout * p.Wout;
#pragma unroll
  for (int a = 0; a < NPB; ++a) {
    const int oy = ty * k.th + wave * RPW + a / XB;
    const int ox = tx * k.tw + (a % XB) * 16 + j;
    if (oy >= p.Hout || ox >= p.Wout) continue;
    const int pix = oy * p.Wout + ox;
#pragma unroll
    for (int m = 0; m < MB; ++m) {
#pragma unroll
      for (int r = 0; r < 4; ++r) {
        const int co = (cog * MB + m) * 16 + 4 * g + r;
        if (co >= k.cout_eff) continue;
        float v = acc[a][m][r];
        if (p.store_mode == 0) {
          if (p.bias) v += p.bias[co];
          if (p.res1.ptr) v += view_ptr(p.res1, b, co, hwout)[pix];
          if (p.res2.ptr) v += view_ptr(p.res2, b, co, hwout)[pix];
          v = act_apply(v, p.act, co);
          if (p.post.ptr) v += view_ptr(p.post, b, co, hwout)[pix];
          p.out[((size_t)b * p.out_ctot + p.out_coff + co) * (size_t)hwout + pix] = v;
        } else {
          const int q = co / p.Cout, c = co - q * p.Cout;
          if (p.bias) v += p.bias[c];
          v = act_apply(v, p.act, c);
          const int W2 = 2 * p.Wout;
          p.out[((size_t)b * p.out_ctot + p.out_coff + c) * (size_t)(4 * hwout) +
                (size_t)(2 * oy + (q >> 1)) * W2 + 2 * ox + (q & 1)] = v;
        }
      }
    }
  }
}

template <int NW, int NPB, int MB, int WREG, int QREG>
__global__ __launch_bounds__(NW * 64) void conv_quad_kernel(const ConvK k) {
  extern __shared__ __attribute__((aligned(16))) float smem[];
  conv_quad_body<NW, NPB, MB, WREG, QREG>(k, k.xcd ? conv_xcd_item(blockIdx.x, gridDim.x) : blockIdx.x, smem);
}

constexpr int CONVQ_MULTI_MAX = 4;
struct ConvKN {
  ConvK k[CONVQ_MULTI_MAX];
  int start[CONVQ_MULTI_MAX + 1];
};
template <int NW, int NPB, int MB, int WREG, int QREG>
__global__ __launch_bounds__(NW * 64) void conv_quad_multi_kernel(const ConvKN kn) {
  extern __shared__ __attribute__((aligned(16))) float smem[];
  const int bid = blockIdx.x;
  if (bid < kn.start[1]) conv_quad_body<NW, NPB, MB, WREG, QREG>(kn.k[0], bid, smem);
  else if (bid < kn.start[2]) conv_quad_body<NW, NPB, MB, WREG, QREG>(kn.k[1], bid - kn.start[1], smem);
  else if (bid < kn.start[3]) conv_quad_body<NW, NPB, MB, WREG, QREG>(kn.k[2], bid - kn.start[2], smem);
  else conv_quad_body<NW, NPB, MB, WREG, QREG>(kn.k[3], bid - kn.start[3], smem);
}

#define CONVQ_GROUP_A(X) X(4, 1, 2, 8, 1) X(4, 1, 2, 16, 2) X(4, 1, 4, 12, 1) X(4, 1, 4, 16, 2) X(4, 1, 1, 8, 2)
#define CONVQ_GROUP_B(X) X(4, 2, 2, 8, 2) X(4, 2, 2, 16, 2) X(4, 2, 4, 12, 2) X(4, 2, 4, 16, 2) X(4, 2, 1, 8, 2)
#define CONVQ_GROUP_C(X) X(9, 1, 2, 8, 1) X(9, 1, 4, 8, 1) X(9, 1, 4, 16, 1) X(9, 1, 1, 8, 1) X(4, 4, 1, 8, 4) X(4, 4, 2, 8, 4)
#define CONVQ_ALL(X) CONVQ_GROUP_A(X) CONVQ_GROUP_B(X) CONVQ_GROUP_C(X)
#define CONVQ_DECLARE(NW, NPB, MB, WREG, QREG) extern template __global__ void conv_quad_kernel<NW, NPB, MB, WREG, QREG>(const ConvK);
#define CONVQ_DEFINE(NW, NPB, MB, WREG, QREG) template __global__ void conv_quad_kernel<NW, NPB, MB, WREG, QREG>(const ConvK);
#define CONVQ_MULTI(X) X(4, 1, 1, 8, 2) X(4, 1, 2, 16, 2)
#define CONVQM_DECLARE(NW, NPB, MB, WREG, QREG) extern template __global__ void conv_quad_multi_kernel<NW, NPB, MB, WREG, QREG>(const ConvKN);
#define CONVQM_DEFINE(NW, NPB, MB, WREG, QREG) template __global__ void conv_quad_multi_kernel<NW, NPB, MB, WREG, QREG>(const ConvKN);
```

### codd_amd/csrc/stereo.hip

```cpp
#include "common.h"
#include <stdlib.h>

#define CV_TPB 16
__global__ __launch_bounds__(256) void costvol_argmin_kernel(const float* __restrict__ L, const float* __restrict__ R,
                                                             int C, int Ht, int Wt, int Wr, int D, float* cost,
                                                             int cost_ctot, int cost_coff, float* disp, int disp_ctot,
                                                             int disp_coff, int zero_dxdy) {
  extern __shared__ float sm[];
  const int tid = threadIdx.x, lane = tid & 63, wave = tid >> 6;
  const int xt0 = blockIdx.x * CV_TPB, y = blockIdx.y, b = blockIdx.z;
  const int win = D + 4 * (CV_TPB - 1);
  const int base = 4 * xt0 - (D - 1);
  float* rl = sm;
  float* ll = sm + C * win;
  const float* Rb = R + ((size_t)b * C * Ht + y) * Wr;
  for (int e = tid; e < C * win; e += 256) {
    const int c = e / win, i = e - c * win, gx = base + i;
    rl[e] = (gx >= 0 && gx < Wr) ? Rb[(size_t)c * Ht * Wr + gx] : 0.f;
  }
  const float* Lb = L + ((size_t)b * C * Ht + y) * Wt;
  for (int e = tid; e < C * CV_TPB; e += 256) {
    const int c = e / CV_TPB, i = e - c * CV_TPB, gx = xt0 + i;
    ll[e] = gx < Wt ? Lb[(size_t)c * Ht * Wt + gx] : 0.f;
  }
  __syncthreads();
  for (int t = wave; t < CV_TPB; t += 4) {
    const int xt = xt0 + t;
    if (xt >= Wt) break;
    float best = INFINITY;
    int bi = 0x7fffffff;
    const int o = 4 * t + (D - 1);
    for (int d = lane; d < D; d += 64) {
      float s = 0.f;
      for (int c = 0; c < C; ++c) s += fabsf(ll[c * CV_TPB + t] - rl[c * win + o - d]);
      if (s < best) { best = s; bi = d; }
    }
#pragma unroll
    for (int off = 32; off > 0; off >>= 1) {
      const float ob = __shfl_xor(best, off, 64);
      const int oi = __shfl_xor(bi, off, 64);
      if (ob < best || (ob == best && oi < bi)) { best = ob; bi = oi; }
    }
    if (lane == 0) {
      const size_t hw = (size_t)Ht * Wt, pix = (size_t)y * Wt + xt;
      cost[((size_t)b * cost_ctot + cost_coff) * hw + pix] = best;
      float* dp = disp + ((size_t)b * disp_ctot + disp_coff) * hw + pix;
      dp[0] = (float)bi;
      if (zero_dxdy) { dp[hw] = 0.f; dp[2 * hw] = 0.f; }
    }
  }
}

template <int TPB>
__global__ __launch_bounds__(256) void costvol_argmin4_kernel(const float* __restrict__ L, const float* __restrict__ R,
                                                              int C, int Ht, int Wt, int Wr, int D, float* cost,
                                                              int cost_ctot, int cost_coff, float* disp, int disp_ctot,
                                                              int disp_coff, int zero_dxdy) {
  extern __shared__ __attribute__((aligned(16))) float sm[];
  const int tid = threadIdx.x, lane = tid & 63, wave = tid >> 6;
  int bx_, y, b;
  codd_xcd_block(bx_, y, b);
  const int xt0 = bx_ * TPB;
  const int win = D + 4 * (TPB - 1);
  const int base = 4 * xt0 - (D - 1);
  float* rl = sm;
  float* ll = sm + C * win;
  const float* Rb = R + ((size_t)b * C * Ht + y) * Wr;
  for (int c = wave; c < C; c += 4) {
    const float* rc = Rb + (size_t)c * Ht * Wr;
    for (int i = lane; i < win; i += 64) {
      const int gx = base + i;
      rl[c * win + i] = (gx >= 0 && gx < Wr) ? rc[gx] : 0.f;
    }
  }
  const float* Lb = L + ((size_t)b * C * Ht + y) * Wt;
  for (int e = tid; e < C * TPB; e += 256) {
    const int c = e / TPB, i = e - c * TPB, gx = xt0 + i;
    ll[e] = gx < Wt ? Lb[(size_t)c * Ht * Wt + gx] : 0.f;
  }
  __syncthreads();
  for (int t0 = 4 * wave; t0 < TPB && xt0 + t0 < Wt; t0 += 16) {
    float best[4];
    int bi[4];
#pragma unroll
    for (int q = 0; q < 4; ++q) { best[q] = INFINITY; bi[q] = 0x7fffffff; }
    for (int d0 = 4 * lane; d0 < D; d0 += 256) {
      float s[4][4];
#pragma unroll
      for (int q = 0; q < 4; ++q)
#pragma unroll
        for (int k = 0; k < 4; ++k) s[q][k] = 0.f;
      const int o = 4 * t0 + D - 4 - d0;
      for (int c = 0; c < C; ++c) {
        const float4 l4 = *(const float4*)(ll + c * TPB + t0);
        const float lv[4] = {l4.x, l4.y, l4.z, l4.w};
#pragma unroll
        for (int q = 0; q < 4; ++q) {
          const float4 r4 = *(const float4*)(rl + c * win + o + 4 * q);
          s[q][3] += fabsf(lv[q] - r4.x);
          s[q][2] += fabsf(lv[q] - r4.y);
          s[q][1] += fabsf(lv[q] - r4.z);
          s[q][0] += fabsf(lv[q] - r4.w);
        }
      }
#pragma unroll
      for (int q = 0; q < 4; ++q)
#pragma unroll
        for (int k = 0; k < 4; ++k)
          if (s[q][k] < best[q]) { best[q] = s[q][k]; bi[q] = d0 + k; }
    }
#pragma unroll
    for (int q = 0; q < 4; ++q) {
      float bb = best[q];
      int ii = bi[q];
#pragma unroll
      for (int off = 32; off > 0; off >>= 1) {
        const float ob = __shfl_xor(bb, off, 64);
        const int oi = __shfl_xor(ii, off, 64);
        if (ob < bb || (ob == bb && oi < ii)) { bb = ob; ii = oi; }
      }
      const int xt = xt0 + t0 + q;
      if (lane == 0 && xt < Wt) {
        const size_t hw = (size_t)Ht * Wt, pix = (size_t)y * Wt + xt;
        cost[((size_t)b * cost_ctot + cost_coff) * hw + pix] = bb;
        float* dp = disp + ((size_t)b * disp_ctot + disp_coff) * hw + pix;
        dp[0] = (float)ii;
        if (zero_dxdy) { dp[hw] = 0.f; dp[2 * hw] = 0.f; }
      }
    }
  }
}

extern "C" int codd_tile_costvol_argmin(const float* L, const float* R, int B, int C, int Ht, int Wt, int Wr, int D,
                                        float* cost, int cost_ctot, int cost_coff, float* disp, int disp_ctot,
                                        int disp_coff, int zero_dxdy, void* stream) {
  if (!L || !R || !cost || !disp || B < 1 || C < 1 || D < 1 || Ht < 1 || Wt < 1) return CODD_EINVAL;
  hipStream_t st = (hipStream_t)stream;
  if ((D & 3) == 0) {
    int tpb = 16;
    for (;; tpb >>= 1) {
      const int win = D + 4 * (tpb - 1);
      const size_t lds = (size_t)(C * win + C * tpb) * sizeof(float);
      if (lds > 64 * 1024) { if (tpb == 16) return CODD_EUNSUPPORTED; continue; }
      dim3 grid(cdiv(Wt, tpb), Ht, B);
#define CV_LAUNCH(T) costvol_argmin4_kernel<T><<<grid, 256, lds, st>>>(L, R, C, Ht, Wt, Wr, D, cost, cost_ctot, cost_coff, disp, disp_ctot, disp_coff, zero_dxdy)
      if (tpb == 64) CV_LAUNCH(64); else if (tpb == 32) CV_LAUNCH(32); else CV_LAUNCH(16);
#undef CV_LAUNCH
      break;
    }
    CODD_LAUNCH_CHECK();
    return CODD_OK;
  }
  const int win = D + 4 * (CV_TPB - 1);
  size_t lds = (size_t)(C * win + C * CV_TPB) * sizeof(float);
  if (lds > 64 * 1024) return CODD_EUNSUPPORTED;
  dim3 grid(cdiv(Wt, CV_TPB), Ht, B);
  costvol_argmin_kernel<<<grid, 256, lds, st>>>(L, R, C, Ht, Wt, Wr, D, cost, cost_ctot, cost_coff,
                                                disp, disp_ctot, disp_coff, zero_dxdy);
  CODD_LAUNCH_CHECK();
  return CODD_OK;
}

template <bool STAGE>
__global__ __launch_bounds__(256) void tile_warp_kernel(const float* __restrict__ fl, const float* __restrict__ fr,
                                                        int C, int Ht, int Wt, codd_view h0, codd_view h1, int nhyp,
                                                        float* out0, float* out1) {
  extern __shared__ __attribute__((aligned(16))) float srow[];
  const int txr = blockIdx.x * blockDim.x + threadIdx.x;
  const int yy = blockIdx.y;
  const int b = blockIdx.z;
  if (!STAGE && txr >= Wt) return;
  const bool live = txr < Wt;
  const int tx = live ? txr : Wt - 1;
  const int ty = yy >> 2, iy = yy & 3;
  const int H = 4 * Ht, W = 4 * Wt;
  if (STAGE) {
    const float4* src = (const float4*)(fr + (size_t)b * C * H * W + (size_t)yy * W);
    const int w4 = W >> 2, chw4 = (H * W) >> 2;
    for (int c = 0; c < C; ++c)
      for (int x4 = threadIdx.x; x4 < w4; x4 += blockDim.x) ((float4*)srow)[c * w4 + x4] = src[(size_t)c * chw4 + x4];
    __syncthreads();
  }
  const size_t thw = (size_t)Ht * Wt, tpix = (size_t)ty * Wt + tx;
  const float* flb = fl + (size_t)b * C * H * W + (size_t)yy * W + 4 * tx;
  const float* frb = fr + (size_t)b * C * H * W + (size_t)yy * W;
  const size_t chw = (size_t)H * W;

  int f0[2][4];
  float a[2][4];
  unsigned okm[2] = {0u, 0u};
#pragma unroll
  for (int hsel = 0; hsel < 2; ++hsel) {
    const codd_view hv = (hsel && nhyp == 2) ? h1 : h0;
    const float* hp = hv.ptr + ((size_t)b * hv.ctot + hv.coff) * thw + tpix;
    const float d = hp[0], dx = hp[thw], dy = hp[2 * thw];
#pragma unroll
    for (int ix = 0; ix < 4; ++ix) {
      const float delta = d + (ix - 1.5f) * dx + (iy - 1.5f) * dy;
      const float xs = (float)(4 * tx + ix) - delta;
      const float fl0 = floorf(xs);
      a[hsel][ix] = xs - fl0;
      f0[hsel][ix] = (int)fminf(fmaxf(fl0, -4.f), (float)W + 4.f);
#pragma unroll
      for (int q = 0; q < 4; ++q)
        if ((unsigned)(f0[hsel][ix] - 1 + q) < (unsigned)W) okm[hsel] |= 1u << (ix * 4 + q);
    }
  }
  float fea[4] = {0.f, 0.f, 0.f, 0.f};
  float cv[2][3][4] = {{{0.f}}};
#pragma unroll 2
  for (int c = 0; c < C; ++c) {
    const float4 l4 = *(const float4*)(flb + c * chw);
    const float lv[4] = {l4.x, l4.y, l4.z, l4.w};
    const float* rr = frb + c * chw;
    float t[2][4][4];
#pragma unroll
    for (int hsel = 0; hsel < 2; ++hsel) {
      if (hsel < nhyp) {
#pragma unroll
        for (int ix = 0; ix < 4; ++ix)
#pragma unroll
          for (int q = 0; q < 4; ++q) {
            const int xi = min(max(f0[hsel][ix] - 1 + q, 0), W - 1);
            t[hsel][ix][q] = STAGE ? srow[c * W + xi] : rr[xi];
          }
      }
    }
#pragma unroll
    for (int ix = 0; ix < 4; ++ix) fea[ix] += fabsf(lv[ix]);
#pragma unroll
    for (int hsel = 0; hsel < 2; ++hsel) {
      if (hsel < nhyp) {
#pragma unroll
        for (int ix = 0; ix < 4; ++ix) {
          float tq[4];
#pragma unroll
          for (int q = 0; q < 4; ++q) tq[q] = (okm[hsel] >> (ix * 4 + q)) & 1u ? t[hsel][ix][q] : 0.f;
          const float w1 = a[hsel][ix], w0 = 1.f - a[hsel][ix];
          cv[hsel][0][ix] += fabsf(lv[ix] - (w0 * tq[2] + w1 * tq[3]));
          cv[hsel][1][ix] += fabsf(lv[ix] - (w0 * tq[1] + w1 * tq[2]));
          cv[hsel][2][ix] += fabsf(lv[ix] - (w0 * tq[0] + w1 * tq[1]));
        }
      }
    }
  }
  if (!live) return;
#pragma unroll
  for (int ix = 0; ix < 4; ++ix) {
    const int ch = iy * 4 + ix;
    const size_t o = (size_t)b * 64 * thw + tpix;
    out0[o + (size_t)ch * thw] = fea[ix];
    if (nhyp == 2) out1[o + (size_t)ch * thw] = fea[ix];
#pragma unroll
    for (int k = 0; k < 3; ++k) {
      out0[o + (size_t)(16 + k * 16 + ch) * thw] = cv[0][k][ix];
      if (nhyp == 2) out1[o + (size_t)(16 + k * 16 + ch) * thw] = cv[1][k][ix];
    }
  }
}

extern "C" int codd_tile_warp_cost(const float* fl, const float* fr, int B, int C, int Ht, int Wt, codd_view hyp0,
                                   codd_view hyp1, int nhyp, float* out0, float* out1, void* stream) {
  if (!fl || !fr || !hyp0.ptr || !out0 || nhyp < 1 || nhyp > 2 || (nhyp == 2 && (!hyp1.ptr || !out1)))
    return CODD_EINVAL;
  const size_t lds = (size_t)C * 4 * Wt * sizeof(float);
  if (lds <= 96 * 1024 && ((uintptr_t)fr & 15) == 0) {
    if (lds > 64 * 1024 &&
        hipFuncSetAttribute((const void*)tile_warp_kernel<true>, hipFuncAttributeMaxDynamicSharedMemorySize, (int)lds) != hipSuccess)
      return CODD_EUNSUPPORTED;
    const int bx = Wt > 128 ? 256 : (Wt > 64 ? 128 : 64);
    dim3 grid(cdiv(Wt, bx), 4 * Ht, B);
    tile_warp_kernel<true><<<grid, bx, lds, (hipStream_t)stream>>>(fl, fr, C, Ht, Wt, hyp0, hyp1, nhyp, out0, out1);
    CODD_LAUNCH_CHECK();
    return CODD_OK;
  }
  const int bx = 64;
  dim3 grid(cdiv(Wt, bx), 4 * Ht, B);
  tile_warp_kernel<false><<<grid, bx, 0, (hipStream_t)stream>>>(fl, fr, C, Ht, Wt, hyp0, hyp1, nhyp, out0, out1);
  CODD_LAUNCH_CHECK();
  return CODD_OK;
}

__global__ void hyp_upsample_kernel(codd_view in, int h, int w, float scale, float* out, int out_ctot, int out_coff,
                                    long long total) {
  long long e = (long long)blockIdx.x * blockDim.x + threadIdx.x;
  if (e >= total) return;
  const int W2 = 2 * w, H2 = 2 * h;
  const int x = (int)(e % W2);
  long long t = e / W2;
  const int y = (int)(t % H2); t /= H2;
  const int c = (int)(t % 16);
  const int b = (int)(t / 16);
  const size_t hw = (size_t)h * w;
  const float* ip = in.ptr + ((size_t)b * in.ctot + in.coff) * hw + (size_t)(y >> 1) * w + (x >> 1);
  float v;
  if (c == 0) {
    const float cx = (x & 1) ? 0.5f : -0.5f, cy = (y & 1) ? 0.5f : -0.5f;
    v = (ip[0] + cx * ip[hw] + cy * ip[2 * hw]) * scale;
  } else {
    v = ip[(size_t)c * hw];
  }
  out[((size_t)b * out_ctot + out_coff + c) * (size_t)(4 * hw) + (size_t)y * W2 + x] = v;
}

extern "C" int codd_hyp_upsample(codd_view in, int B, int h, int w, float scale, float* out, int out_ctot,
                                 int out_coff, void* stream) {
  if (!in.ptr || !out) return CODD_EINVAL;
  long long total = (long long)B * 16 * 4 * h * w;
  hyp_upsample_kernel<<<cdiv(total, 256), 256, 0, (hipStream_t)stream>>>(in, h, w, scale, out, out_ctot, out_coff,
                                                                         total);
  CODD_LAUNCH_CHECK();
  return CODD_OK;
}

__global__ void hyp_select_kernel(const float* __restrict__ upd, codd_view cur, codd_view prev, int hw, float* out,
                                  int out_ctot, int out_coff, long long total) {
  long long e = (long long)blockIdx.x * blockDim.x + threadIdx.x;
  if (e >= total) return;
  const int pix = (int)(e % hw);
  long long t = e / hw;
  const int c = (int)(t % 16);
  const int b = (int)(t / 16);
  const float* u = upd + (size_t)b * 34 * hw + pix;
  const bool sel_cur = u[hw] > u[0];
  float v;
  if (sel_cur) v = cur.ptr[((size_t)b * cur.ctot + cur.coff + c) * hw + pix] + u[(size_t)(18 + c) * hw];
  else v = prev.ptr[((size_t)b * prev.ctot + prev.coff + c) * hw + pix] + u[(size_t)(2 + c) * hw];
  if (c == 0) v = fmaxf(v, 0.f);
  out[((size_t)b * out_ctot + out_coff + c) * hw + pix] = v;
}

extern "C" int codd_hyp_select(const float* upd, codd_view cur, codd_view prev, int B, int h, int w, float* out,
                               int out_ctot, int out_coff, void* stream) {
  if (!upd || !cur.ptr || !prev.ptr || !out) return CODD_EINVAL;
  long long total = (long long)B * 16 * h * w;
  hyp_select_kernel<<<cdiv(total, 256), 256, 0, (hipStream_t)stream>>>(upd, cur, prev, h * w, out, out_ctot, out_coff,
                                                                       total);
  CODD_LAUNCH_CHECK();
  return CODD_OK;
}

extern "C" int codd_abi_version(void) { return CODD_ABI_VERSION; }

static int g_opt[CODD_OPT_COUNT] = {192, 5};
int codd_opt(int key) { return g_opt[key]; }
extern "C" int codd_get_option(int key) { return key >= 0 && key < CODD_OPT_COUNT ? g_opt[key] : CODD_EINVAL; }
extern "C" int codd_set_option(int key, int value) {
  if (key < 0 || key >= CODD_OPT_COUNT) return CODD_EINVAL;
  if (key == CODD_OPT_GN_Q4 && (value < 16 || value > 4096)) return CODD_EINVAL;
  if (key == CODD_OPT_GN_BUILDER && value != 3 && value != 5) return CODD_EINVAL;
  const int prev = g_opt[key];
  g_opt[key] = value;
  return prev;
}
```

### include/codd_hip.h

```cpp
#ifndef CODD_HIP_H
#define CODD_HIP_H

#ifdef __cplusplus
extern "C" {
#endif

#define CODD_ABI_VERSION 12

#define CODD_OK 0
#define CODD_EINVAL (-1)
#define CODD_EUNSUPPORTED (-2)

enum { CODD_OPT_GN_Q4 = 0, CODD_OPT_GN_BUILDER = 1, CODD_OPT_COUNT = 2 };
int codd_set_option(int key, int value);
int codd_get_option(int key);

enum { CODD_ACT_NONE = 0, CODD_ACT_LRELU02 = 1, CODD_ACT_RELU = 2, CODD_ACT_SIGMOID = 3,
       CODD_ACT_TANH = 4, CODD_ACT_MISH = 5, CODD_ACT_RELU_CH0 = 6 };

typedef struct {
  const float* ptr;
  int ctot;
  int coff;
} codd_view;

#define CODD_TERMS_BF16 1
#define CODD_TERMS_SPLIT 3
#define CODD_TERMS_F16 16
#define CODD_TERMS_SPLIT_F16 48
#define CODD_TERMS_OK(t) ((t) == 1 || (t) == 3 || (t) == 16 || (t) == 48)
#define CODD_TERMS_PLANES(t) (((t) == 3 || (t) == 48) ? 2 : 1)
#define CODD_TERMS_IS_F16(t) ((t) == 16 || (t) == 48)
typedef struct codd_xs_view {
  void* ptr;
  int c8, hp, wp, bt, bl, o8, terms;
} codd_xs_view;

typedef struct {
  codd_view in0, in1;
  int C0, C1;
  int B, Hin, Win;
  const float* wpacked;
  const float* bias;
  codd_view res1, res2, post;
  float* out;
  int out_ctot, out_coff;
  int Cout, Hout, Wout;
  int kh, kw, sy, sx, pad_t, pad_l, dil_y, dil_x;
  int act;
  int store_mode;
  int mb;
  int npb;
  int nw;
  int ck;
  int layout;
  int terms;
  int pgw, cgw;
  const void* xs;
  int xs_c8, xs_hp, xs_wp;
  int xs_bt, xs_bl;
  int xs_o8;
  void* xso;
  int xso_c8, xso_hp, xso_wp, xso_bt, xso_bl, xso_o8, xso_terms;
  int ksplit;
  int dil2;
  int gate;
} codd_conv_params;

int codd_conv2d(const codd_conv_params* p, void* stream);
int codd_conv2d_multi(const codd_conv_params* p, int n, void* stream);
int codd_conv2d_check(const codd_conv_params* p);

long long codd_conv2d_packed_size_quad(int Cout, int Cin, int kh, int kw, int mb, int ck);
int codd_conv2d_pack_weights_quad(const float* w, float* wpacked, int Cout, int Cin, int kh, int kw, int mb,
                                  int ck, void* stream);

long long codd_split_bf16_bytes(int B, int c8, int hp, int wp, int terms);
int codd_split_bf16(codd_view in0, int C0, codd_view in1, int C1, int B, int H, int W, int bt, int bl,
                    int c8, int hp, int wp, int terms, void* xs, void* stream);

long long codd_conv2d_packed_bytes_bf16(int Cout, int Cin, int kh, int kw, int mb, int ck, int terms);
int codd_conv2d_pack_weights_bf16(const float* w, void* wpacked, int Cout, int Cin, int kh, int kw, int mb, int ck,
                                  int terms, long long co_stride, long long ci_stride, float scale, void* stream);

long long codd_conv2d_packed_size(int Cout, int Cin, int kh, int kw, int mb, int ck);
int codd_conv2d_pack_weights(const float* w, float* wpacked, int Cout, int Cin, int kh, int kw,
                             int mb, int ck, void* stream);
int codd_conv2d_pack_weights_ex(const float* w, float* wpacked, int Cout, int Cin, int kh, int kw,
                                int mb, int ck, long long co_stride, long long ci_stride, float scale,
                                void* stream);

typedef struct {
  codd_view in0, in1;
  int C0, C1;
  int B, H, W;
  int C;
  int mode;
  const float* wA;
  const float* bA;
  const float* wB;
  const float* bB;
  int actA, actB;
  int residual;
  float* out;
  int out_ctot, out_coff, cout_store;
  int rh;
} codd_roll_params;
long long codd_roll_packed_size(int C, int k, int Cin);
int codd_roll_pack_weights(const float* w, float* packed, int C, int Cout, int Cin, int k, void* stream);
int codd_conv_roll(const codd_roll_params* p, void* stream);

int codd_tile_costvol_argmin(const float* L, const float* R, int B, int C, int Ht, int Wt, int Wr, int D,
                             float* cost, int cost_ctot, int cost_coff,
                             float* disp, int disp_ctot, int disp_coff, int zero_dxdy, void* stream);

int codd_tile_warp_cost(const float* fl, const float* fr, int B, int C, int Ht, int Wt,
                        codd_view hyp0, codd_view hyp1, int nhyp,
                        float* out0, float* out1, void* stream);

int codd_hyp_upsample(codd_view in, int B, int h, int w, float scale,
                      float* out, int out_ctot, int out_coff, void* stream);

int codd_hyp_select(const float* upd, codd_view cur, codd_view prev, int B, int h, int w,
                    float* out, int out_ctot, int out_coff, void* stream);

int codd_instnorm(const float* x, int B, int C, int HW, float* stats, const float* res, int relu,
                  float* y, void* stream);
int codd_instnorm_xs(const float* x, int B, int C, int H, int W, float* stats, const float* res, int relu,
                     int relu_after_res, float* y, codd_xs_view xs, void* stream);

int codd_allpairs_corr(const float* f1, const float* f2, int B, int D, int h, int w,
                       float* lvl0, float* lvl1, float* lvl2, float* lvl3, float* scratch, void* stream);
long long codd_allpairs_corr_scratch(int B, int D, int h, int w);
int codd_avgpool2(const float* in, int BC, int h, int w, float* out, void* stream);

int codd_corr_lookup(const float* lvl0, const float* lvl1, const float* lvl2, const float* lvl3,
                     const float* coords, int cstride, int B, int h, int w, float* out, void* stream);

int codd_raft_geometry(const float* T, const float* depth1, const float* depth2, int B, int h, int w,
                       float fx, float fy, float cx, float cy, float* xyz, float* minfo, void* stream);

long long codd_se3_gn_scratch(int B, int h, int w, int radius);
int codd_se3_gn_step(float* T, const float* ae, int ae_c, const float* xyz, const float* delta,
                     const float* weight, const float* depth1, int B, int h, int w,
                     float fx, float fy, float cx, float cy, int radius, float lm, float ep,
                     float* Hb, void* stream);

int codd_se3_gn_step_heads(float* T, codd_xs_view hidden, const void* head_w, const float* head_b,
                           const float* xyz, const float* depth1, int B, int h, int w, float fx, float fy,
                           float cx, float cy, int radius, float lm, float ep, float* weight_out, float* Hb,
                           void* stream);

int codd_cvx_upsample(const float* data, const float* mask, int B, int h, int w, int dim, int mode,
                      float* out, void* stream);
int codd_cvx_upsample_se3_weight(const float* T, const float* weight, const float* mask, int B, int h, int w,
                                 float* T_out, float* weight_out, void* stream);

int codd_disp_to_depth(const float* disp, long long n, float bf, float* depth, void* stream);
int codd_subsample(const float* in, int B, int H, int W, int oy, int ox, int step, float* out, void* stream);

long long codd_splat_scratch(int B, int H, int W, float radius);
int codd_splat(const float* T, const float* depth, int HT, int WT, int oy, int ox, int ds,
               const float* featA, int CA, const float* featB, int CB, int with_flow,
               int B, int H, int W, float fx, float fy, float cx, float cy, float radius,
               float bf, float* out, float* zout, int* scratch, void* stream);

int codd_induced_flow(const float* T, const float* depth, int B, int H, int W,
                      float fx, float fy, float cx, float cy, float* out, void* stream);

int codd_context_split(const float* x, int B, int hw, float* net, float* inp, void* stream);

int codd_se3_identity(float* T, long long npix, void* stream);

int codd_resize_bilinear(const float* in, int B, int C, int Hi, int Wi, int Ho, int Wo, int align_corners,
                         float* out, int out_ctot, int out_coff, int accumulate, int relu, void* stream);
int codd_resize_bilinear_add(const float* in, int B, int C, int Hi, int Wi, int Ho, int Wo, int align_corners,
                             float* out, int out_ctot, int out_coff, int accumulate, int relu, const float* extra,
                             void* stream);

int codd_add_relu(const float* a, const float* b, long long n, int relu, float* y, void* stream);
int codd_copy_many(const float* const* src, float* const* dst, const long long* n, int count, void* stream);

int codd_timestamp(long long* slot, void* stream);

int codd_gru_gate_zr(const float* t1, const float* t2, const float* inp, const float* cor,
                     const float* mot, const float* h, int B, int hw, float* zr, float* rh, void* stream);
int codd_gru_gate_q(const float* t1, const float* t2, const float* inp, const float* cor,
                    const float* mot, const float* zr, const float* h, int B, int hw, float* hout,
                    void* stream);


int codd_gru_gate_zr_xs(const float* t1, const float* t2, const float* inp, const float* cor, const float* mot,
                        const float* h, int B, int H, int W, float* z, codd_xs_view rh_xs, void* stream);
int codd_gru_gate_q_xs(const float* t1, const float* t2, const float* inp, const float* cor, const float* mot,
                       const float* z, const float* h, int B, int H, int W, float* hout, codd_xs_view h_xs,
                       void* stream);

int codd_fusion_cues_lr(const float* pred_curr, const float* pred_warp, const float* feat_curr,
                        const float* feat_warp, const float* fea_l, const float* fea_r,
                        int B, int H, int W, int patch, int ds, int CF, int CS, float* corr_feat,
                        float* dsub, int dsub_ctot, int dsub_coff, void* stream);

int codd_fusion_cues_fr(const float* pred_curr, const float* pred_warp, const float* flow_warp,
                        const float* conf_warp, int B, int H, int W, int patch, float* out, void* stream);

int codd_fusion_forget(const float* pred_curr, const float* pred_warp, const float* flow_warp,
                       const float* conf_warp, int B, int H, int W, int patch, const float* weff, float* wr,
                       void* stream);

int codd_fusion_blend(const float* pred_curr, const float* pred_warp, const float* wf_lr,
                      const float* wr_logit_sig, int B, int H, int W, int ds,
                      float* fused, float* wf_out, float* wr_out, void* stream);

int codd_disp_metrics(const float* pred, const float* gt, int B, int H, int W, int h, int w,
                      float lo, float hi, float thr, double* scratch, double* meters, void* stream);

int codd_tepe_metrics(const float* pred, const float* gt, const float* pred_prev, const float* gt_prev,
                      const float* flow_prev, const float* gt_mask, const float* gt2_prev, int B, int H, int W,
                      int h, int w, float lo, float hi, float bf, double* scratch, double* meters, void* stream);

int codd_sceneflow_metrics(const float* Ts, const float* pred_prev, const float* gt_disp_prev,
                           const float* gt_flow_prev, const float* gt_disp_change, const unsigned char* gt_flow_occ,
                           int B, int H, int W, int h, int w, float lo, float hi, float bf, float fx, float fy,
                           float cx, float cy, double* scratch, double* meters, void* stream);

int codd_preprocess(const unsigned char* img, int h, int w, int bgr, const float* mean, const float* stdv,
                    int H, int W, float* out, void* stream);

int codd_fusion_select(int mode, const float* cur, const float* warp, const float* gt, int B, int H,
                       int W, int hg, int wg, float K, float* out, void* stream);
int codd_gt_motion(const float* img_prev, const float* disp_prev, const float* feat_prev, int C,
                   const float* gt_flow, const float* gt_disp_change, const unsigned char* gt_flow_occ,
                   int B, int H, int W, int hg, int wg, float* img_warp, float* feat_warp, float* conf,
                   float* disp_warp, float* flow3, void* stream);

int codd_raft_geometry_lookup(const float* T, const float* depth1, const float* depth2, const float* lvl0,
                              const float* lvl1, const float* lvl2, const float* lvl3, int B, int h, int w,
                              float fx, float fy, float cx, float cy, float* xyz, float* minfo, float* out,
                              void* stream);
int codd_raft_geometry_lookup_xs(const float* T, const float* depth1, const float* depth2, const float* lvl0,
                                 const float* lvl1, const float* lvl2, const float* lvl3, int B, int h, int w,
                                 float fx, float fy, float cx, float cy, float* xyz, codd_xs_view minfo_xs,
                                 codd_xs_view corr_xs, void* stream);

int codd_abi_version(void);

#ifdef __cplusplus
}
#endif
#endif
```

Measured before the change: 105.9 frames/s.

## Add double-buffered DMA ring staging to quad f32 conv kernel

Adds a ring-staged variant of the quad (f32 MFMA) convolution kernel. Weights are loaded straight into LDS via global_load_lds DMA, and when LDS allows, two buffers let the next chunk's weights and inputs load while the current chunk computes. The inner loop is also software-pipelined so the LDS reads for the next step are issued before the MFMAs of the current one. The new path is the default through a new option, and it doubles LDS use per block, which can reduce occupancy.

```diff
diff --git a/codd_amd/_abi.py b/codd_amd/_abi.py
--- a/codd_amd/_abi.py
+++ b/codd_amd/_abi.py
@@ -174,7 +174,7 @@
     return lib
 
 
-OPTIONS = dict(gn_q4=0, gn_builder=1)
+OPTIONS = dict(gn_q4=0, gn_builder=1, quad_staging=2)
 
 
 def set_option(name, value):
diff --git a/codd_amd/csrc/conv.hip b/codd_amd/csrc/conv.hip
--- a/codd_amd/csrc/conv.hip
+++ b/codd_amd/csrc/conv.hip
@@ -112,14 +112,14 @@
   return CODD_EUNSUPPORTED;
 }
 
-template <int NW, int NPB, int MB, int WREG, int QREG>
+template <int NW, int NPB, int MB, int WREG, int QREG, bool RING>
 static int launch_quad(const ConvK& k, size_t lds, int grid, hipStream_t s) {
   if (lds > 64 * 1024) {
-    hipError_t e = hipFuncSetAttribute((const void*)conv_quad_kernel<NW, NPB, MB, WREG, QREG>,
+    hipError_t e = hipFuncSetAttribute((const void*)conv_quad_kernel<NW, NPB, MB, WREG, QREG, RING>,
                                        hipFuncAttributeMaxDynamicSharedMemorySize, (int)lds);
     if (e != hipSuccess) return (int)e;
   }
-  conv_quad_kernel<NW, NPB, MB, WREG, QREG><<<grid, NW * 64, lds, s>>>(k);
+  conv_quad_kernel<NW, NPB, MB, WREG, QREG, RING><<<grid, NW * 64, lds, s>>>(k);
   CODD_LAUNCH_CHECK();
   return CODD_OK;
 }
@@ -127,7 +127,9 @@
 static int launch_quad_any(const ConvK& k, int nw, size_t lds, int grid, hipStream_t s) {
   const codd_conv_params& p = k.p;
   const int nt = nw * 64, wr = cdiv(k.wchunk >> 2, nt), qr = cdiv((p.ck >> 2) * k.upc, nt);
-#define Q(W, N, M, R, QQ) if (nw == W && p.npb == N && p.mb == M && wr <= R && qr <= QQ) return launch_quad<W, N, M, R, QQ>(k, lds, grid, s);
+#define Q(W, N, M, R, QQ)                                                                                \
+  if (nw == W && p.npb == N && p.mb == M && wr <= R && qr <= QQ)                                         \
+    return k.nring ? launch_quad<W, N, M, R, QQ, true>(k, lds, grid, s) : launch_quad<W, N, M, R, QQ, false>(k, lds, grid, s);
   Q(4, 1, 1, 8, 2) Q(4, 1, 2, 8, 1) Q(4, 1, 2, 16, 2) Q(4, 1, 4, 12, 1) Q(4, 1, 4, 16, 2)
   Q(4, 2, 1, 8, 2) Q(4, 2, 2, 8, 2) Q(4, 2, 2, 16, 2) Q(4, 2, 4, 12, 2) Q(4, 2, 4, 16, 2)
   Q(4, 4, 1, 8, 4) Q(4, 4, 2, 8, 4)
@@ -142,6 +144,8 @@
   if (!pp || pp->layout != 2) return CODD_EINVAL;
   return codd_conv2d_bf16(pp, nullptr, 1);
 }
+
+#define QUAD_RING_LDS_MAX (40 * 1024)
 
 static int conv_fill(const codd_conv_params* pp, ConvK& k, size_t& lds, long long& grid, int& nw) {
   k.p = *pp;
@@ -179,10 +183,15 @@
   k.vec_ok = (p.Win % 4 == 0) && ((uintptr_t)p.in0.ptr % 16 == 0) && (hwb % 16 == 0) &&
              (p.C1 == 0 || (uintptr_t)p.in1.ptr % 16 == 0);
   lds = ((size_t)k.wchunk + (size_t)p.ck * k.chs) * sizeof(float);
+  k.nring = 0;
   if (p.layout == 1) {
     if (!(p.ck == 16 || p.ck == 32) || p.sx > 2 || !k.vec_ok) return CODD_EUNSUPPORTED;
     k.wchunk = k.ntaps * p.ck * 16 * p.mb;
     lds = ((size_t)k.wchunk + (size_t)p.ck * k.thi * k.twp) * sizeof(float);
+    if (codd_opt(CODD_OPT_QUAD_STAGING) == 2) {
+      if (k.nchunks == 1) k.nring = 1;
+      else if (2 * lds <= QUAD_RING_LDS_MAX) { k.nring = 2; lds *= 2; }
+    }
   } else if (p.layout != 0) {
     return CODD_EINVAL;
   }
@@ -224,14 +233,14 @@
   return CODD_EUNSUPPORTED;
 }
 
-template <int NW, int NPB, int MB, int WREG, int QREG>
+template <int NW, int NPB, int MB, int WREG, int QREG, bool RING>
 static int launch_quad_multi(const ConvKN& kn, size_t lds, int grid, hipStream_t s) {
   if (lds > 64 * 1024) {
-    hipError_t e = hipFuncSetAttribute((const void*)conv_quad_multi_kernel<NW, NPB, MB, WREG, QREG>,
+    hipError_t e = hipFuncSetAttribute((const void*)conv_quad_multi_kernel<NW, NPB, MB, WREG, QREG, RING>,
                                        hipFuncAttributeMaxDynamicSharedMemorySize, (int)lds);
     if (e != hipSuccess) return (int)e;
   }
-  conv_quad_multi_kernel<NW, NPB, MB, WREG, QREG><<<grid, NW * 64, lds, s>>>(kn);
+  conv_quad_multi_kernel<NW, NPB, MB, WREG, QREG, RING><<<grid, NW * 64, lds, s>>>(kn);
   CODD_LAUNCH_CHECK();
   return CODD_OK;
 }
@@ -241,9 +250,10 @@
   if (n == 1) return codd_conv2d(ps, stream);
   ConvKN kn;
   memset(&kn, 0, sizeof(kn));
-  size_t lds = 0;
+  size_t lds = 0, lds1 = 0;
   long long total = 0;
   int wr = 0, qr = 0;
+  bool ring = true;
   for (int i = 0; i < n; ++i) {
     size_t l;
     long long g;
@@ -257,14 +267,25 @@
     wr = w_ > wr ? w_ : wr;
     qr = q_ > qr ? q_ : qr;
     lds = l > lds ? l : lds;
+    const size_t l1 = kn.k[i].nring == 2 ? l / 2 : l;
+    lds1 = l1 > lds1 ? l1 : lds1;
+    ring = ring && kn.k[i].nring;
     kn.start[i] = (int)total;
     total += g;
   }
   for (int i = n; i <= CONVQ_MULTI_MAX; ++i) kn.start[i] = (int)total;
   if (total > 0x7fffffffLL) return CODD_EINVAL;
+  if (!ring) {
+    for (int i = 0; i < n; ++i) kn.k[i].nring = 0;
+    lds = lds1;
+  }
   hipStream_t s = (hipStream_t)stream;
-  if (ps[0].mb == 1 && wr <= 8 && qr <= 2) return launch_quad_multi<4, 1, 1, 8, 2>(kn, lds, (int)total, s);
-  if (ps[0].mb == 2 && wr <= 16 && qr <= 2) return launch_quad_multi<4, 1, 2, 16, 2>(kn, lds, (int)total, s);
+#define QM(M, R, QQ)                                                                                     \
+  if (ps[0].mb == M && wr <= R && qr <= QQ)                                                              \
+    return ring ? launch_quad_multi<4, 1, M, R, QQ, true>(kn, lds, (int)total, s)                         \
+                : launch_quad_multi<4, 1, M, R, QQ, false>(kn, lds, (int)total, s);
+  QM(1, 8, 2) QM(2, 16, 2)
+#undef QM
   return CODD_EUNSUPPORTED;
 }
 
diff --git a/codd_amd/csrc/conv_bf16_kernel.h b/codd_amd/csrc/conv_bf16_kernel.h
--- a/codd_amd/csrc/conv_bf16_kernel.h
+++ b/codd_amd/csrc/conv_bf16_kernel.h
@@ -146,12 +146,6 @@
 #undef CONVB_W1
 }
 
-__device__ __forceinline__ void convb_dma16(const uint4* gsrc, unsigned lds_dst) {
-  unsigned keep;
-  asm volatile("s_mov_b32 %0, m0\n\ts_mov_b32 m0, %2\n\ts_nop 0\n\tglobal_load_lds_dwordx4 %1, off\n\ts_mov_b32 m0, %0"
-               : "=&s"(keep) : "v"(gsrc), "s"(lds_dst) : "memory");
-}
-
 template <int I, int NR, int NM>
 struct ConvbSched {
   static __device__ __forceinline__ void run() {
diff --git a/codd_amd/csrc/conv_kernel.h b/codd_amd/csrc/conv_kernel.h
--- a/codd_amd/csrc/conv_kernel.h
+++ b/codd_amd/csrc/conv_kernel.h
@@ -17,6 +17,7 @@
   int upc;
   int nunits;
   int vec_ok;
+  int nring;
   int xcd;
 };
 
@@ -27,6 +28,12 @@
 
 __device__ __forceinline__ const float* view_ptr(const codd_view& v, int b, int c, int hw) {
   return v.ptr + ((size_t)b * v.ctot + v.coff + c) * (size_t)hw;
+}
+
+__device__ __forceinline__ void convb_dma16(const uint4* gsrc, unsigned lds_dst) {
+  unsigned keep;
+  asm volatile("s_mov_b32 %0, m0\n\ts_mov_b32 m0, %2\n\ts_nop 0\n\tglobal_load_lds_dwordx4 %1, off\n\ts_mov_b32 m0, %0"
+               : "=&s"(keep) : "v"(gsrc), "s"(lds_dst) : "memory");
 }
 
 template <int NW, int NPB, int MB, int WREG, int IREG>
diff --git a/codd_amd/csrc/conv_quad_kernel.h b/codd_amd/csrc/conv_quad_kernel.h
--- a/codd_amd/csrc/conv_quad_kernel.h
+++ b/codd_amd/csrc/conv_quad_kernel.h
@@ -1,135 +1,12 @@
 #pragma once
 #include "conv_kernel.h"
 
-template <int NW, int NPB, int MB, int WREG, int QREG>
-__device__ __forceinline__ void conv_quad_body(const ConvK& k, int bid, float* smem) {
-  constexpr int NT = NW * 64;
-  float* wl = smem;
-  float* il = smem + k.wchunk;
+template <int NPB, int MB>
+__device__ __forceinline__ void conv_quad_store(const ConvK& k, const f32x4 (&acc)[NPB][MB], int tx, int ty, int cog, int b,
+                                                int wave, int g, int j) {
   const codd_conv_params& p = k.p;
-  const int tid = threadIdx.x, lane = tid & 63, wave = tid >> 6;
-  const int g = lane >> 4, j = lane & 15;
   constexpr int XB = NPB >= 2 ? 2 : 1;
   constexpr int RPW = NPB / XB;
-
-  const int tx = bid % k.tiles_x; bid /= k.tiles_x;
-  const int ty = bid % k.tiles_y; bid /= k.tiles_y;
-  const int cog = bid % k.ncog;
-  const int b = bid / k.ncog;
-
-  const int hwin = p.Hin * p.Win;
-  const int gy0 = ty * k.th * p.sy - p.pad_t;
-  const int gxs = tx * k.tw * p.sx - p.pad_l - k.xoff;
-
-  const int ncq = p.ck >> 2;
-  const int nq = ncq * k.upc;
-  int q_lds[QREG], q_g[QREG], q_c[QREG];
-  bool q_in[QREG];
-#pragma unroll
-  for (int r = 0; r < QREG; ++r) {
-    const int u = tid + r * NT;
-    q_c[r] = -1; q_in[r] = false; q_lds[r] = 0; q_g[r] = 0;
-    if (u < nq) {
-      const int cq = u / k.upc, rem = u - cq * k.upc;
-      const int y = rem / k.twp4, x4 = rem - y * k.twp4;
-      const int gy = gy0 + y, gx = gxs + 4 * x4;
-      q_c[r] = 4 * cq;
-      q_in[r] = (unsigned)gy < (unsigned)p.Hin && gx >= 0 && gx + 3 < p.Win;
-      q_lds[r] = ((cq * k.thi + y) * k.twp + 4 * x4) * 4;
-      q_g[r] = gy * p.Win + gx;
-    }
-  }
-  const int wchunk4 = k.wchunk >> 2;
-  float4 wreg[WREG], ireg[QREG][4];
-
-#define QUAD_ISSUE(CH)                                                                                    \
-  {                                                                                                       \
-    const float4* src_ = (const float4*)(p.wpacked + ((size_t)(cog * k.nchunks + (CH))) * k.wchunk);      \
-    _Pragma("unroll") for (int r = 0; r < WREG; ++r) {                                                    \
-      const int e = tid + r * NT;                                                                         \
-      wreg[r] = e < wchunk4 ? src_[e] : make_float4(0.f, 0.f, 0.f, 0.f);                                  \
-    }                                                                                                     \
-    _Pragma("unroll") for (int r = 0; r < QREG; ++r) {                                                    \
-      _Pragma("unroll") for (int c = 0; c < 4; ++c) {                                                     \
-        float4 v = make_float4(0.f, 0.f, 0.f, 0.f);                                                       \
-        const int cg = (CH) * p.ck + q_c[r] + c;                                                          \
-        if (q_c[r] >= 0 && q_in[r] && cg < k.cin) {                                                       \
-          const float* s_ =                                                                               \
-              (cg < p.C0 ? view_ptr(p.in0, b, cg, hwin) : view_ptr(p.in1, b, cg - p.C0, hwin)) + q_g[r];  \
-          v = *(const float4*)s_;                                                                         \
-        }                                                                                                 \
-        ireg[r][c] = v;                                                                                   \
-      }                                                                                                   \
-    }                                                                                                     \
-  }
-#define QUAD_COMMIT()                                                                                     \
-  {                                                                                                       \
-    float4* dst_ = (float4*)wl;                                                                           \
-    _Pragma("unroll") for (int r = 0; r < WREG; ++r) {                                                    \
-      const int e = tid + r * NT;                                                                         \
-      if (e < wchunk4) dst_[e] = wreg[r];                                                                 \
-    }                                                                                                     \
-    _Pragma("unroll") for (int r = 0; r < QREG; ++r) if (q_c[r] >= 0) {                                   \
-      float4* d_ = (float4*)(il + q_lds[r]);   \
-      d_[0] = make_float4(ireg[r][0].x, ireg[r][1].x, ireg[r][2].x, ireg[r][3].x);                        \
-      d_[1] = make_float4(ireg[r][0].y, ireg[r][1].y, ireg[r][2].y, ireg[r][3].y);                        \
-      d_[2] = make_float4(ireg[r][0].z, ireg[r][1].z, ireg[r][2].z, ireg[r][3].z);                        \
-      d_[3] = make_float4(ireg[r][0].w, ireg[r][1].w, ireg[r][2].w, ireg[r][3].w);                        \
-    }                                                                                                     \
-  }
-
-  f32x4 acc[NPB][MB];
-#pragma unroll
-  for (int a = 0; a < NPB; ++a)
-#pragma unroll
-    for (int m = 0; m < MB; ++m) acc[a][m] = (f32x4){0.f, 0.f, 0.f, 0.f};
-
-  int pbase[NPB];
-#pragma unroll
-  for (int a = 0; a < NPB; ++a) {
-    const int prow = wave * RPW + a / XB, pcol = (a % XB) * 16 + j;
-    pbase[a] = prow * p.sy * k.twp + pcol * p.sx + k.xoff;
-  }
-  const int wq = 16 * MB;
-  const int iq = k.thi * k.twp;
-  const int ngr = p.ck >> 4;
-
-  QUAD_ISSUE(0);
-  for (int ch = 0; ch < k.nchunks; ++ch) {
-    __syncthreads();
-    QUAD_COMMIT();
-    __syncthreads();
-    if (ch + 1 < k.nchunks) QUAD_ISSUE(ch + 1);
-    const float4* w4 = (const float4*)wl;
-    const float4* i4 = (const float4*)il;
-    for (int ky = 0; ky < p.kh; ++ky) {
-      for (int kx = 0; kx < p.kw; ++kx) {
-        const float4* wp = w4 + ((size_t)(ky * p.kw + kx) * (p.ck >> 2) + g) * wq + j;
-        const float4* ip = i4 + (size_t)g * iq + ky * p.dil_y * k.twp + kx * p.dil_x;
-        for (int gr = 0; gr < ngr; ++gr) {
-          float4 av[MB], bv[NPB];
-#pragma unroll
-          for (int m = 0; m < MB; ++m) av[m] = wp[m * 16];
-#pragma unroll
-          for (int a = 0; a < NPB; ++a) bv[a] = ip[pbase[a]];
-          wp += 4 * wq;
-          ip += 4 * iq;
-#pragma unroll
-          for (int a = 0; a < NPB; ++a)
-#pragma unroll
-            for (int m = 0; m < MB; ++m) {
-              acc[a][m] = __builtin_amdgcn_mfma_f32_16x16x4f32(av[m].x, bv[a].x, acc[a][m], 0, 0, 0);
-              acc[a][m] = __builtin_amdgcn_mfma_f32_16x16x4f32(av[m].y, bv[a].y, acc[a][m], 0, 0, 0);
-              acc[a][m] = __builtin_amdgcn_mfma_f32_16x16x4f32(av[m].z, bv[a].z, acc[a][m], 0, 0, 0);
-              acc[a][m] = __builtin_amdgcn_mfma_f32_16x16x4f32(av[m].w, bv[a].w, acc[a][m], 0, 0, 0);
-            }
-        }
-      }
-    }
-  }
-#undef QUAD_ISSUE
-#undef QUAD_COMMIT
-
   const int hwout = p.Hout * p.Wout;
 #pragma unroll
   for (int a = 0; a < NPB; ++a) {
@@ -165,9 +42,311 @@
 }
 
 template <int NW, int NPB, int MB, int WREG, int QREG>
+__device__ __forceinline__ void conv_quad_body(const ConvK& k, int bid, float* smem) {
+  constexpr int NT = NW * 64;
+  float* wl = smem;
+  float* il = smem + k.wchunk;
+  const codd_conv_params& p = k.p;
+  const int tid = threadIdx.x, lane = tid & 63, wave = tid >> 6;
+  const int g = lane >> 4, j = lane & 15;
+  constexpr int XB = NPB >= 2 ? 2 : 1;
+  constexpr int RPW = NPB / XB;
+
+  const int tx = bid % k.tiles_x; bid /= k.tiles_x;
+  const int ty = bid % k.tiles_y; bid /= k.tiles_y;
+  const int cog = bid % k.ncog;
+  const int b = bid / k.ncog;
+
+  const int hwin = p.Hin * p.Win;
+  const int gy0 = ty * k.th * p.sy - p.pad_t;
+  const int gxs = tx * k.tw * p.sx - p.pad_l - k.xoff;
+
+  const int ncq = p.ck >> 2;
+  const int nq = ncq * k.upc;
+  int q_lds[QREG], q_g[QREG], q_c[QREG];
+  bool q_in[QREG];
+#pragma unroll
+  for (int r = 0; r < QREG; ++r) {
+    const int u = tid + r * NT;
+    q_c[r] = -1; q_in[r] = false; q_lds[r] = 0; q_g[r] = 0;
+    if (u < nq) {
+      const int cq = u / k.upc, rem = u - cq * k.upc;
+      const int y = rem / k.twp4, x4 = rem - y * k.twp4;
+      const int gy = gy0 + y, gx = gxs + 4 * x4;
+      q_c[r] = 4 * cq;
+      q_in[r] = (unsigned)gy < (unsigned)p.Hin && gx >= 0 && gx + 3 < p.Win;
+      q_lds[r] = ((cq * k.thi + y) * k.twp + 4 * x4) * 4;
+      q_g[r] = gy * p.Win + gx;
+    }
+  }
+  const int wchunk4 = k.wchunk >> 2;
+  float4 wreg[WREG], ireg[QREG][4];
+
+#define QUAD_ISSUE(CH)                                                                                    \
+  {                                                                                                       \
+    const float4* src_ = (const float4*)(p.wpacked + ((size_t)(cog * k.nchunks + (CH))) * k.wchunk);      \
+    _Pragma("unroll") for (int r = 0; r < WREG; ++r) {                                                    \
+      const int e = tid + r * NT;                                                                         \
+      wreg[r] = e < wchunk4 ? src_[e] : make_float4(0.f, 0.f, 0.f, 0.f);                                  \
+    }                                                                                                     \
+    _Pragma("unroll") for (int r = 0; r < QREG; ++r) {                                                    \
+      _Pragma("unroll") for (int c = 0; c < 4; ++c) {                                                     \
+        float4 v = make_float4(0.f, 0.f, 0.f, 0.f);                                                       \
+        const int cg = (CH) * p.ck + q_c[r] + c;                                                          \
+        if (q_c[r] >= 0 && q_in[r] && cg < k.cin) {                                                       \
+          const float* s_ =                                                                               \
+              (cg < p.C0 ? view_ptr(p.in0, b, cg, hwin) : view_ptr(p.in1, b, cg - p.C0, hwin)) + q_g[r];  \
+          v = *(const float4*)s_;                                                                         \
+        }                                                                                                 \
+        ireg[r][c] = v;                                                                                   \
+      }                                                                                                   \
+    }                                                                                                     \
+  }
+#define QUAD_COMMIT()                                                                                     \
+  {                                                                                                       \
+    float4* dst_ = (float4*)wl;                                                                           \
+    _Pragma("unroll") for (int r = 0; r < WREG; ++r) {                                                    \
+      const int e = tid + r * NT;                                                                         \
+      if (e < wchunk4) dst_[e] = wreg[r];                                                                 \
+    }                                                                                                     \
+    _Pragma("unroll") for (int r = 0; r < QREG; ++r) if (q_c[r] >= 0) {                                   \
+      float4* d_ = (float4*)(il + q_lds[r]);   \
+      d_[0] = make_float4(ireg[r][0].x, ireg[r][1].x, ireg[r][2].x, ireg[r][3].x);                        \
+      d_[1] = make_float4(ireg[r][0].y, ireg[r][1].y, ireg[r][2].y, ireg[r][3].y);                        \
+      d_[2] = make_float4(ireg[r][0].z, ireg[r][1].z, ireg[r][2].z, ireg[r][3].z);                        \
+      d_[3] = make_float4(ireg[r][0].w, ireg[r][1].w, ireg[r][2].w, ireg[r][3].w);                        \
+    }                                                                                                     \
+  }
+
+  f32x4 acc[NPB][MB];
+#pragma unroll
+  for (int a = 0; a < NPB; ++a)
+#pragma unroll
+    for (int m = 0; m < MB; ++m) acc[a][m] = (f32x4){0.f, 0.f, 0.f, 0.f};
+
+  int pbase[NPB];
+#pragma unroll
+  for (int a = 0; a < NPB; ++a) {
+    const int prow = wave * RPW + a / XB, pcol = (a % XB) * 16 + j;
+    pbase[a] = prow * p.sy * k.twp + pcol * p.sx + k.xoff;
+  }
+  const int wq = 16 * MB;
+  const int iq = k.thi * k.twp;
+  const int ngr = p.ck >> 4;
+
+  QUAD_ISSUE(0);
+  for (int ch = 0; ch < k.nchunks; ++ch) {
+    __syncthreads();
+    QUAD_COMMIT();
+    __syncthreads();
+    if (ch + 1 < k.nchunks) QUAD_ISSUE(ch + 1);
+    const float4* w4 = (const float4*)wl;
+    const float4* i4 = (const float4*)il;
+    for (int ky = 0; ky < p.kh; ++ky) {
+      for (int kx = 0; kx < p.kw; ++kx) {
+        const float4* wp = w4 + ((size_t)(ky * p.kw + kx) * (p.ck >> 2) + g) * wq + j;
+        const float4* ip = i4 + (size_t)g * iq + ky * p.dil_y * k.twp + kx * p.dil_x;
+        for (int gr = 0; gr < ngr; ++gr) {
+          float4 av[MB], bv[NPB];
+#pragma unroll
+          for (int m = 0; m < MB; ++m) av[m] = wp[m * 16];
+#pragma unroll
+          for (int a = 0; a < NPB; ++a) bv[a] = ip[pbase[a]];
+          wp += 4 * wq;
+          ip += 4 * iq;
+#pragma unroll
+          for (int a = 0; a < NPB; ++a)
+#pragma unroll
+            for (int m = 0; m < MB; ++m) {
+              acc[a][m] = __builtin_amdgcn_mfma_f32_16x16x4f32(av[m].x, bv[a].x, acc[a][m], 0, 0, 0);
+              acc[a][m] = __builtin_amdgcn_mfma_f32_16x16x4f32(av[m].y, bv[a].y, acc[a][m], 0, 0, 0);
+              acc[a][m] = __builtin_amdgcn_mfma_f32_16x16x4f32(av[m].z, bv[a].z, acc[a][m], 0, 0, 0);
+              acc[a][m] = __builtin_amdgcn_mfma_f32_16x16x4f32(av[m].w, bv[a].w, acc[a][m], 0, 0, 0);
+            }
+        }
+      }
+    }
+  }
+#undef QUAD_ISSUE
+#undef QUAD_COMMIT
+
+  conv_quad_store<NPB, MB>(k, acc, tx, ty, cog, b, wave, g, j);
+}
+
+template <int NW, int NPB, int MB, int QREG>
+__device__ __forceinline__ void conv_quad_ring_body(const ConvK& k, int bid, float* smem) {
+  constexpr int NT = NW * 64;
+  const codd_conv_params& p = k.p;
+  const int tid = threadIdx.x, lane = tid & 63, wave = tid >> 6;
+  const int g = lane >> 4, j = lane & 15;
+  constexpr int XB = NPB >= 2 ? 2 : 1;
+  constexpr int RPW = NPB / XB;
+
+  const int tx = bid % k.tiles_x; bid /= k.tiles_x;
+  const int ty = bid % k.tiles_y; bid /= k.tiles_y;
+  const int cog = bid % k.ncog;
+  const int b = bid / k.ncog;
+
+  const int hwin = p.Hin * p.Win;
+  const int gy0 = ty * k.th * p.sy - p.pad_t;
+  const int gxs = tx * k.tw * p.sx - p.pad_l - k.xoff;
+
+  const int ncq = p.ck >> 2;
+  const int nq = ncq * k.upc;
+  int q_lds[QREG], q_g[QREG], q_c[QREG];
+  bool q_in[QREG];
+#pragma unroll
+  for (int r = 0; r < QREG; ++r) {
+    const int u = tid + r * NT;
+    q_c[r] = -1; q_in[r] = false; q_lds[r] = 0; q_g[r] = 0;
+    if (u < nq) {
+      const int cq = u / k.upc, rem = u - cq * k.upc;
+      const int y = rem / k.twp4, x4 = rem - y * k.twp4;
+      const int gy = gy0 + y, gx = gxs + 4 * x4;
+      q_c[r] = 4 * cq;
+      q_in[r] = (unsigned)gy < (unsigned)p.Hin && gx >= 0 && gx + 3 < p.Win;
+      q_lds[r] = ((cq * k.thi + y) * k.twp + 4 * x4) * 4;
+      q_g[r] = gy * p.Win + gx;
+    }
+  }
+  const int bufsz = k.wchunk + p.ck * k.thi * k.twp;
+  const int nwp = k.wchunk >> 8;
+  const unsigned smem_lds = (unsigned)(uintptr_t)(__attribute__((address_space(3))) float*)smem;
+  const uint4* wsrc = (const uint4*)(p.wpacked + (size_t)cog * k.nchunks * k.wchunk) + lane;
+  float4 ireg[QREG][4];
+
+#define RING_DMA_W(CH, BUF)                                                                               \
+  {                                                                                                       \
+    const uint4* src_ = wsrc + (size_t)(CH) * (k.wchunk >> 2);                                            \
+    const unsigned dst_ = smem_lds + (unsigned)((BUF) * bufsz) * 4u;                                      \
+    for (int i_ = wave; i_ < nwp; i_ += NW)                                                               \
+      convb_dma16(src_ + i_ * 64, __builtin_amdgcn_readfirstlane(dst_ + (unsigned)i_ * 1024u));           \
+  }
+#define RING_ISSUE_I(CH)                                                                                  \
+  {                                                                                                       \
+    _Pragma("unroll") for (int r = 0; r < QREG; ++r) {                                                    \
+      _Pragma("unroll") for (int c = 0; c < 4; ++c) {                                                     \
+        float4 v = make_float4(0.f, 0.f, 0.f, 0.f);                                                       \
+        const int cg = (CH) * p.ck + q_c[r] + c;                                                          \
+        if (q_c[r] >= 0 && q_in[r] && cg < k.cin) {                                                       \
+          const float* s_ =                                                                               \
+              (cg < p.C0 ? view_ptr(p.in0, b, cg, hwin) : view_ptr(p.in1, b, cg - p.C0, hwin)) + q_g[r];  \
+          v = *(const float4*)s_;                                                                         \
+        }                                                                                                 \
+        ireg[r][c] = v;                                                                                   \
+      }                                                                                                   \
+    }                                                                                                     \
+  }
+#define RING_COMMIT_I(BUF)                                                                                \
+  {                                                                                                       \
+    float* il_ = smem + (BUF) * bufsz + k.wchunk;                                                         \
+    _Pragma("unroll") for (int r = 0; r < QREG; ++r) if (q_c[r] >= 0) {                                   \
+      float4* d_ = (float4*)(il_ + q_lds[r]);                                                             \
+      d_[0] = make_float4(ireg[r][0].x, ireg[r][1].x, ireg[r][2].x, ireg[r][3].x);                        \
+      d_[1] = make_float4(ireg[r][0].y, ireg[r][1].y, ireg[r][2].y, ireg[r][3].y);                        \
+      d_[2] = make_float4(ireg[r][0].z, ireg[r][1].z, ireg[r][2].z, ireg[r][3].z);                        \
+      d_[3] = make_float4(ireg[r][0].w, ireg[r][1].w, ireg[r][2].w, ireg[r][3].w);                        \
+    }                                                                                                     \
+  }
+#define RING_LANDED_BARRIER()                                                                             \
+  {                                                                                                       \
+    asm volatile("s_waitcnt vmcnt(0)" ::: "memory");                                                      \
+    __syncthreads();                                                                                      \
+  }
+
+  f32x4 acc[NPB][MB];
+#pragma unroll
+  for (int a = 0; a < NPB; ++a)
+#pragma unroll
+    for (int m = 0; m < MB; ++m) acc[a][m] = (f32x4){0.f, 0.f, 0.f, 0.f};
+
+  int pbase[NPB];
+#pragma unroll
+  for (int a = 0; a < NPB; ++a) {
+    const int prow = wave * RPW + a / XB, pcol = (a % XB) * 16 + j;
+    pbase[a] = prow * p.sy * k.twp + pcol * p.sx + k.xoff;
+  }
+  const int wq = 16 * MB;
+  const int iq = k.thi * k.twp;
+  const int ngr = p.ck >> 4;
+  const int nsteps = k.ntaps * ngr;
+
+  RING_DMA_W(0, 0);
+  RING_ISSUE_I(0);
+  RING_COMMIT_I(0);
+  RING_LANDED_BARRIER();
+  for (int ch = 0; ch < k.nchunks; ++ch) {
+    const int cur = k.nring == 2 ? (ch & 1) : 0, nxt = k.nring == 2 ? cur ^ 1 : 0;
+    const bool more = ch + 1 < k.nchunks;
+    if (more) {
+      if (k.nring == 2) RING_DMA_W(ch + 1, nxt);
+      RING_ISSUE_I(ch + 1);
+    }
+    const float4* wp = (const float4*)(smem + cur * bufsz) + g * wq + j;
+    const float4* ib = (const float4*)(smem + cur * bufsz + k.wchunk) + g * iq;
+    int gr = 0, ky = 0, kx = 0, toff = 0;
+    float4 av[MB], bv[NPB];
+#pragma unroll
+    for (int m = 0; m < MB; ++m) av[m] = wp[m * 16];
+#pragma unroll
+    for (int a = 0; a < NPB; ++a) bv[a] = ib[pbase[a]];
+    for (int t = 0; t < nsteps; ++t) {
+      if (t + 1 < nsteps) {
+        wp += 4 * wq;
+        if (++gr == ngr) {
+          gr = 0;
+          if (++kx == p.kw) { kx = 0; ++ky; }
+          toff = ky * p.dil_y * k.twp + kx * p.dil_x;
+        }
+      }
+      const float4* ip = ib + gr * 4 * iq + toff;
+      float4 an[MB], bn[NPB];
+#pragma unroll
+      for (int m = 0; m < MB; ++m) an[m] = wp[m * 16];
+#pragma unroll
+      for (int a = 0; a < NPB; ++a) bn[a] = ip[pbase[a]];
+      __builtin_amdgcn_sched_barrier(0);
+#pragma unroll
+      for (int a = 0; a < NPB; ++a)
+#pragma unroll
+        for (int m = 0; m < MB; ++m) {
+          acc[a][m] = __builtin_amdgcn_mfma_f32_16x16x4f32(av[m].x, bv[a].x, acc[a][m], 0, 0, 0);
+          acc[a][m] = __builtin_amdgcn_mfma_f32_16x16x4f32(av[m].y, bv[a].y, acc[a][m], 0, 0, 0);
+          acc[a][m] = __builtin_amdgcn_mfma_f32_16x16x4f32(av[m].z, bv[a].z, acc[a][m], 0, 0, 0);
+          acc[a][m] = __builtin_amdgcn_mfma_f32_16x16x4f32(av[m].w, bv[a].w, acc[a][m], 0, 0, 0);
+        }
+#pragma unroll
+      for (int m = 0; m < MB; ++m) av[m] = an[m];
+#pragma unroll
+      for (int a = 0; a < NPB; ++a) bv[a] = bn[a];
+    }
+    if (more) {
+      if (k.nring != 2) {
+        __syncthreads();
+        RING_DMA_W(ch + 1, 0);
+      }
+      RING_COMMIT_I(nxt);
+      RING_LANDED_BARRIER();
+    }
+  }
+#undef RING_DMA_W
+#undef RING_ISSUE_I
+#undef RING_COMMIT_I
+#undef RING_LANDED_BARRIER
+
+  conv_quad_store<NPB, MB>(k, acc, tx, ty, cog, b, wave, g, j);
+}
+
+template <int NW, int NPB, int MB, int WREG, int QREG, bool RING>
+__device__ __forceinline__ void conv_quad_any_body(const ConvK& k, int bid, float* smem) {
+  if constexpr (RING) conv_quad_ring_body<NW, NPB, MB, QREG>(k, bid, smem);
+  else conv_quad_body<NW, NPB, MB, WREG, QREG>(k, bid, smem);
+}
+
+template <int NW, int NPB, int MB, int WREG, int QREG, bool RING>
 __global__ __launch_bounds__(NW * 64) void conv_quad_kernel(const ConvK k) {
   extern __shared__ __attribute__((aligned(16))) float smem[];
-  conv_quad_body<NW, NPB, MB, WREG, QREG>(k, k.xcd ? conv_xcd_item(blockIdx.x, gridDim.x) : blockIdx.x, smem);
+  conv_quad_any_body<NW, NPB, MB, WREG, QREG, RING>(k, k.xcd ? conv_xcd_item(blockIdx.x, gridDim.x) : blockIdx.x, smem);
 }
 
 constexpr int CONVQ_MULTI_MAX = 4;
@@ -175,22 +354,30 @@
   ConvK k[CONVQ_MULTI_MAX];
   int start[CONVQ_MULTI_MAX + 1];
 };
-template <int NW, int NPB, int MB, int WREG, int QREG>
+template <int NW, int NPB, int MB, int WREG, int QREG, bool RING>
 __global__ __launch_bounds__(NW * 64) void conv_quad_multi_kernel(const ConvKN kn) {
   extern __shared__ __attribute__((aligned(16))) float smem[];
   const int bid = blockIdx.x;
-  if (bid < kn.start[1]) conv_quad_body<NW, NPB, MB, WREG, QREG>(kn.k[0], bid, smem);
-  else if (bid < kn.start[2]) conv_quad_body<NW, NPB, MB, WREG, QREG>(kn.k[1], bid - kn.start[1], smem);
-  else if (bid < kn.start[3]) conv_quad_body<NW, NPB, MB, WREG, QREG>(kn.k[2], bid - kn.start[2], smem);
-  else conv_quad_body<NW, NPB, MB, WREG, QREG>(kn.k[3], bid - kn.start[3], smem);
+  if (bid < kn.start[1]) conv_quad_any_body<NW, NPB, MB, WREG, QREG, RING>(kn.k[0], bid, smem);
+  else if (bid < kn.start[2]) conv_quad_any_body<NW, NPB, MB, WREG, QREG, RING>(kn.k[1], bid - kn.start[1], smem);
+  else if (bid < kn.start[3]) conv_quad_any_body<NW, NPB, MB, WREG, QREG, RING>(kn.k[2], bid - kn.start[2], smem);
+  else conv_quad_any_body<NW, NPB, MB, WREG, QREG, RING>(kn.k[3], bid - kn.start[3], smem);
 }
 
 #define CONVQ_GROUP_A(X) X(4, 1, 2, 8, 1) X(4, 1, 2, 16, 2) X(4, 1, 4, 12, 1) X(4, 1, 4, 16, 2) X(4, 1, 1, 8, 2)
 #define CONVQ_GROUP_B(X) X(4, 2, 2, 8, 2) X(4, 2, 2, 16, 2) X(4, 2, 4, 12, 2) X(4, 2, 4, 16, 2) X(4, 2, 1, 8, 2)
 #define CONVQ_GROUP_C(X) X(9, 1, 2, 8, 1) X(9, 1, 4, 8, 1) X(9, 1, 4, 16, 1) X(9, 1, 1, 8, 1) X(4, 4, 1, 8, 4) X(4, 4, 2, 8, 4)
 #define CONVQ_ALL(X) CONVQ_GROUP_A(X) CONVQ_GROUP_B(X) CONVQ_GROUP_C(X)
-#define CONVQ_DECLARE(NW, NPB, MB, WREG, QREG) extern template __global__ void conv_quad_kernel<NW, NPB, MB, WREG, QREG>(const ConvK);
-#define CONVQ_DEFINE(NW, NPB, MB, WREG, QREG) template __global__ void conv_quad_kernel<NW, NPB, MB, WREG, QREG>(const ConvK);
+#define CONVQ_DECLARE(NW, NPB, MB, WREG, QREG)                                                             \
+  extern template __global__ void conv_quad_kernel<NW, NPB, MB, WREG, QREG, false>(const ConvK);              \
+  extern template __global__ void conv_quad_kernel<NW, NPB, MB, WREG, QREG, true>(const ConvK);
+#define CONVQ_DEFINE(NW, NPB, MB, WREG, QREG)                                                              \
+  template __global__ void conv_quad_kernel<NW, NPB, MB, WREG, QREG, false>(const ConvK);                     \
+  template __global__ void conv_quad_kernel<NW, NPB, MB, WREG, QREG, true>(const ConvK);
 #define CONVQ_MULTI(X) X(4, 1, 1, 8, 2) X(4, 1, 2, 16, 2)
-#define CONVQM_DECLARE(NW, NPB, MB, WREG, QREG) extern template __global__ void conv_quad_multi_kernel<NW, NPB, MB, WREG, QREG>(const ConvKN);
-#define CONVQM_DEFINE(NW, NPB, MB, WREG, QREG) template __global__ void conv_quad_multi_kernel<NW, NPB, MB, WREG, QREG>(const ConvKN);
+#define CONVQM_DECLARE(NW, NPB, MB, WREG, QREG)                                                            \
+  extern template __global__ void conv_quad_multi_kernel<NW, NPB, MB, WREG, QREG, false>(const ConvKN);       \
+  extern template __global__ void conv_quad_multi_kernel<NW, NPB, MB, WREG, QREG, true>(const ConvKN);
+#define CONVQM_DEFINE(NW, NPB, MB, WREG, QREG)                                                             \
+  template __global__ void conv_quad_multi_kernel<NW, NPB, MB, WREG, QREG, false>(const ConvKN);              \
+  template __global__ void conv_quad_multi_kernel<NW, NPB, MB, WREG, QREG, true>(const ConvKN);
diff --git a/codd_amd/csrc/stereo.hip b/codd_amd/csrc/stereo.hip
--- a/codd_amd/csrc/stereo.hip
+++ b/codd_amd/csrc/stereo.hip
@@ -342,13 +342,14 @@
 
 extern "C" int codd_abi_version(void) { return CODD_ABI_VERSION; }
 
-static int g_opt[CODD_OPT_COUNT] = {192, 5};
+static int g_opt[CODD_OPT_COUNT] = {192, 5, 2};
 int codd_opt(int key) { return g_opt[key]; }
 extern "C" int codd_get_option(int key) { return key >= 0 && key < CODD_OPT_COUNT ? g_opt[key] : CODD_EINVAL; }
 extern "C" int codd_set_option(int key, int value) {
   if (key < 0 || key >= CODD_OPT_COUNT) return CODD_EINVAL;
   if (key == CODD_OPT_GN_Q4 && (value < 16 || value > 4096)) return CODD_EINVAL;
   if (key == CODD_OPT_GN_BUILDER && value != 3 && value != 5) return CODD_EINVAL;
+  if (key == CODD_OPT_QUAD_STAGING && value != 1 && value != 2) return CODD_EINVAL;
   const int prev = g_opt[key];
   g_opt[key] = value;
   return prev;
diff --git a/include/codd_hip.h b/include/codd_hip.h
--- a/include/codd_hip.h
+++ b/include/codd_hip.h
@@ -11,7 +11,7 @@
 #define CODD_EINVAL (-1)
 #define CODD_EUNSUPPORTED (-2)
 
-enum { CODD_OPT_GN_Q4 = 0, CODD_OPT_GN_BUILDER = 1, CODD_OPT_COUNT = 2 };
+enum { CODD_OPT_GN_Q4 = 0, CODD_OPT_GN_BUILDER = 1, CODD_OPT_QUAD_STAGING = 2, CODD_OPT_COUNT = 3 };
 int codd_set_option(int key, int value);
 int codd_get_option(int key);
 
```

After: 106.1 frames/s (median of 6 runs). About the same (+0.1%).
